# kekeblom/DeepCGP

Measured on AMD Instinct MI355X. Metric: ELBO steps/sec (batch=32) + achieved HBM GB/s on K_uf, MNIST M=256 1-layer, higher is better.
Workload: dtype f64; 1 GPU; cfg2_mnist_CH_M256; variant=conv layer + head, M=256, per_gpu_batch=32, global_batch=32, num_samples=10, layers=2, noise=device Philox RNG, dedup_layer0=False, parallelism=image-sharded x1, no collective

## Files before the change

### deepcgp_amd/csrc/common.h

```cpp
#pragma once
#include <hip/hip_runtime.h>
#include <cstdint>
#include <cstdio>
#include <map>
#include <string>
#include <vector>

#include "../../include/dcgp.h"
#include "dev_guard.h"
#include "fused_plan.h"

typedef double d4 __attribute__((ext_vector_type(4)));

static inline int round_up(int x, int m) { return (x + m - 1) / m * m; }
static inline long round_up_l(long x, long m) { return (x + m - 1) / m * m; }
long col_ld(long columns);

struct TimingAcc {
  int launches = 0;
  double ms = 0.0;
};
struct PendingEvent {
  std::string name;
  hipEvent_t start, stop;
};

struct DcgpOptions {
  long no_fused_layer = 0;
  long fused_large = 0;
  long fused_shape = -1;
  long fused_split = -1;
  long fused_persist = -1;
  long fused_pre = -1;
  long fused_parts = -1;
  long fused_rep_share = -1;
  long head_ride = -1;
  long fused_wgs = 0;
  long fused_stagger = -1;
  long kl_side = 0;
  long sweep_no_rows = 0;
  long kl_no_ride = 0;
  long no_fused_bwd = 0;
  long fused_bwd_min_cols = -1;
  long fused_bwd_frags = 0;
  long gemm_tile = 0;
  long grad_no_keep_k = 0;
  long grad_late_kl = 0;
  long head_unfused = 0;
  long no_side_stream = 0;
  long cu_partition = 0;
  long grad_nofork = 0;
  long head_no_overlap = 0;
  long no_factor_reuse = 0;
  long prep_on_chain = 0;
  long no_early_sweep = 0;
  long chain_no_iso = 0;
  long comm_inline = 0;
  long no_rhs_ride = 0;
  long kuf_upw = 0;
  long kuf_split = -1;
  long kuf_wpg = 0;
  long kuf_stream = 0;
  long kuf_no_rep = 0;
  long grad_dz_main = 0;
  long no_syrk = 0;
  long head_upw = 0;
  long share_kb = 0;
  long sweep_occ = -1;
  long head_tail = -1;
  long fused_abl = 0, rb_mixed = 0;
};
long* dcgp_option_slot(DcgpOptions* o, const char* name);
bool dcgp_poison(const char* name = nullptr);
size_t dcgp_guard_bytes();
struct dcgp_ctx;
hipError_t dev_alloc(dcgp_ctx* ctx, void** p, size_t bytes, const char* label);
void dev_free(dcgp_ctx* ctx, void* p);

struct dcgp_ctx {
  int device = 0;
  int n_cus = 256;
  hipStream_t stream = nullptr;
  hipStream_t stream2 = nullptr;
  hipStream_t stream2b = nullptr;
  hipStream_t stream_aux = nullptr;
  hipStream_t stream_comm = nullptr;
  hipEvent_t ev_comm[4] = {};
  int* comm_gate = nullptr;
  hipStream_t stream_m = nullptr, stream2_m = nullptr;
  hipStream_t last_main = nullptr;
  hipEvent_t ev_last = nullptr;
  bool ev_last_valid = false;
  hipEvent_t ev_fork = nullptr, ev_kl = nullptr;
  DcgpOptions opt;
  bool no_side = false;
  hipEvent_t ev_kl2 = nullptr, ev_kl3 = nullptr;
  hipEvent_t ev_g[6] = {};
  hipEvent_t ev_aux = nullptr, ev_aux2 = nullptr;
  std::string err;
  int last_head_rows = 0; long head_ride_launches = 0;
  unsigned fused_head_epoch = 0;
  unsigned fused_pre_epoch = 0;
  std::string ws_tag;
  std::map<std::string, std::pair<void*, size_t>> ws;
  dev_guard::Registry guards;
  bool timing = false;
  int timing_mode = 0;
  unsigned timing_sample = 0;
  std::map<std::string, TimingAcc> tim;
  std::vector<PendingEvent> pending;
  std::vector<hipEvent_t> event_pool;
  double* h_scratch = nullptr;
  int* h_info = nullptr;
  fused_plan::Plan last_fused_plan;
  long long* fused_trace = nullptr;
  std::string sweep_trace_family;
  long long* sweep_trace = nullptr; long sweep_trace_wgs = 0;
  void* comm = nullptr;
  int nranks = 1, rank = 0;
};

int ctx_fail(dcgp_ctx* ctx, int code, const char* fmt, ...);
void* ws_get(dcgp_ctx* ctx, const std::string& name, size_t bytes);
void timing_flush(dcgp_ctx* ctx);

#define HIP_TRY(ctx, call)                                                               \
  do {                                                                                   \
    hipError_t e_ = (call);                                                              \
    if (e_ != hipSuccess)                                                                \
      return ctx_fail((ctx), DCGP_ERR_HIP, "%s failed: %s (%s:%d)", #call, hipGetErrorString(e_), \
                      __FILE__, __LINE__);                                               \
  } while (0)

#define DCGP_TRY(call)        \
  do {                        \
    int s_ = (call);          \
    if (s_ != DCGP_OK) return s_; \
  } while (0)

#define LAUNCH_CHECK(ctx)                                                                \
  do {                                                                                   \
    hipError_t e_ = hipGetLastError();                                                   \
    if (e_ != hipSuccess)                                                                \
      return ctx_fail((ctx), DCGP_ERR_HIP, "kernel launch failed: %s (%s:%d)",           \
                      hipGetErrorString(e_), __FILE__, __LINE__);                        \
  } while (0)

struct ScopedTimer {
  dcgp_ctx* ctx;
  bool on;
  PendingEvent pe;
  ScopedTimer(dcgp_ctx* c, const char* name);
  ~ScopedTimer();
};


struct GemmArgs {
  const double* Wt = nullptr; long wBatch = 0; int ldw = 0;
  const double* B = nullptr;  long bBatch = 0; int ldb = 0;
  double* C = nullptr;        long cBatch = 0; int ldc = 0;
  double* colsq = nullptr;    long sBatch = 0; long sRowBlk = 0;
  const double* cscale = nullptr; long csCol = 0, csBatch = 0; double calpha = 1.0;
  int Mi = 0, Mk = 0, Kc = 0;
  int nW = 1, nB = 1;
  int tri = 0;
  int b_lower = 0;
  int rb_major = 0;
};
int gemm_tn(dcgp_ctx* ctx, const GemmArgs& a, int* n_row_blocks_out);
int gemm_row_block(int Mi, int Kc, int batch);

__device__ __forceinline__ double exp_sweep(double x) {
  const double kf = rint(x * 1.4426950408889634074);
  double r = fma(-kf, 6.93147180369123816490e-01, x);
  r = fma(-kf, 1.90821492927058770002e-10, r);
  double p = 1.6059043836821613e-10;
#define DCGP_EXP_STEP(c) asm("v_fma_f64 %0, %1, %2, %3" : "=v"(p) : "v"(p), "v"(r), "s"((double)(c)))
  DCGP_EXP_STEP(2.08767569878681e-09);
  DCGP_EXP_STEP(2.505210838544172e-08);
  DCGP_EXP_STEP(2.755731922398589e-07);
  DCGP_EXP_STEP(2.7557319223985893e-06);
  DCGP_EXP_STEP(2.48015873015873e-05);
  DCGP_EXP_STEP(1.984126984126984e-04);
// ... 192 lines not shown
```

### deepcgp_amd/csrc/conv_fused.hip

```cpp
#include <cstring>
#include <tuple>

#include "fused_plan.h"
#include "head_units_dev.h"
#include "layer.h"
#include "rng.h"

namespace {

typedef unsigned int u32x2 __attribute__((ext_vector_type(2)));
#define CF_SB __builtin_amdgcn_sched_barrier(0)
#define CF_DW 2
#define CF_P1 50
#define CF_P2 75
#define CF_P3 90
constexpr int CF_D_DEFAULT = 3;

__device__ __forceinline__ void set_prio(int p) {
  switch (p) {
    case 0: __builtin_amdgcn_s_setprio(0); break;
    case 1: __builtin_amdgcn_s_setprio(1); break;
    case 2: __builtin_amdgcn_s_setprio(2); break;
    default: __builtin_amdgcn_s_setprio(3); break;
  }
}
__device__ __forceinline__ int fdiv(int i, int d, float inv_d) {
  int q = (int)(((float)i + 0.5f) * inv_d);
  const int r = i - (int)__umul24((unsigned)q, (unsigned)d);
  return q + (r >= d ? 1 : 0) - (r < 0 ? 1 : 0);
}
__device__ __forceinline__ int frag_of(int w, int W, int c) { return (c >> 1) * 2 * W + ((c & 1) ? 2 * W - 1 - w : w); }

#define CF_TR(k) \
  if (tr_slot >= 0 && lane == 0) a.trace[(tr_slot * 16 + wave) * 16 + (k)] = (long long)__builtin_readcyclecounter();

template <int FN, int NS, int MAXF, int NT, int BTP, int ABL = 0, int HEAD = 0>
__global__ __launch_bounds__(NT) void conv_fused_kernel(ConvFusedArgs a_in) {
  constexpr int BT = BTP == 1 ? 1 : (BTP == 3 ? 2 : (BTP == 4 ? 3 : 0));
  typedef const __attribute__((address_space(4))) ConvFusedArgs KArgs;
  KArgs* ap = (KArgs*)__builtin_amdgcn_kernarg_segment_ptr();
  KArgs& a = *ap;
  constexpr int BN = FN * 16, W = NT / 64, TW = W / NS, FNS = FN / NS, KG = W / FN;
  static_assert(FN % NS == 0 && W % NS == 0 && W % FN == 0, "team split");
  constexpr int CF_D = ((ABL & 4) ? 2 : 0) + (NT >= 1024 ? CF_DW : CF_D_DEFAULT);
  extern __shared__ __attribute__((aligned(16))) double smem[];

  int cu_word = -1;
  if (a.persist && a.cu_slots) {
    int* word = reinterpret_cast<int*>(smem);
    if (threadIdx.x == 0) {
      unsigned xcc, hwid;
      asm volatile("s_getreg_b32 %0, hwreg(HW_REG_XCC_ID)" : "=s"(xcc));
      asm volatile("s_getreg_b32 %0, hwreg(HW_REG_HW_ID)" : "=s"(hwid));
      cu_word = (int)(((xcc & 7u) << 7) | ((hwid >> 8) & 0x7fu));
      word[0] = atomicAdd(a.cu_slots + cu_word, 1);
    }
    __syncthreads();
    const int arrival = word[0];
    __syncthreads();
    if ((arrival & 1) && a.stagger > 0) {
      const long long t0 = wall_clock64();
      while (wall_clock64() - t0 < a.stagger) __builtin_amdgcn_s_sleep(64);
    }
  }
  int strip_next = blockIdx.x;
  if (HEAD || a.pre_n > 0) {
    int* tk = reinterpret_cast<int*>(smem);
    if (threadIdx.x == 0) tk[0] = atomicAdd(a.dyn, 1);
    __syncthreads();
    strip_next = __builtin_amdgcn_readfirstlane(tk[0]);
    __syncthreads();
  }
  const int first_limit = HEAD ? a.n_items + a.head_n : (a.pre_n > 0 ? a.n_items : 0x7fffffff);
  for (int it = 0; strip_next < first_limit; ++it) {
  int tid = threadIdx.x;
  asm volatile("" : "+s"(ap), "+v"(tid));
  KArgs& a = *ap;
  if constexpr (HEAD) {
    if (strip_next >= a.n_items) {
      int* tk = reinterpret_cast<int*>(smem + a.lds_main + a.lds_img + BN);
      const int row = strip_next - a.n_items;
      if (tid == 0) {
        const int s_hi = (row * a.P + a.P - 1) / BN;
        int ok = 1;
        for (int st = (row * a.P) / BN; st <= s_hi && ok; ++st) {
          ok = 0;
          for (int spin = 0; spin < (1 << 24) && !ok; ++spin) {
            ok = __hip_atomic_load(a.head_flag + st, __ATOMIC_RELAXED, __HIP_MEMORY_SCOPE_AGENT) == a.head_epoch ? 1 : 0;
            if (!ok) __builtin_amdgcn_s_sleep(2);
          }
        }
        tk[1] = ok;
      }
      __syncthreads();
      if (tk[1]) {
        head_units_dev::head_units_body<0, 50, 0, NT, true>(ap->head, row);
      } else {
        for (int m = tid; m < a.head.kzx_rows; m += NT) a.head.kzx[(long)m * a.head.ldk + row] = __builtin_nan("");
      }
      if (tid == 0) tk[0] = atomicAdd(a.dyn, 1);
      __syncthreads();
      strip_next = __builtin_amdgcn_readfirstlane(tk[0]);
      if (strip_next >= first_limit) break;
      continue;
    }
  }
  const int Mp = a.Mp, nf = Mp >> 4, R = a.R;
  const int lane = tid & 63, lrow = lane >> 4, lcol = lane & 15;
  const int wave = __builtin_amdgcn_readfirstlane(tid >> 6);
  const int wm = wave % TW, sp = NS == 1 ? 0 : wave / TW;
  double* strip = smem;
  double* aux = smem + a.lds_main;
  double* xn = aux + a.lds_img;
  int* ticket = reinterpret_cast<int*>(xn + BN);
  int* koff = reinterpret_cast<int*>(xn + BN + 2);
  const int jmax = a.Kc - 1;
  int nfw = 0;
#pragma unroll
  for (int c = 0; c < MAXF; ++c) nfw += frag_of(wm, TW, c) < nf ? 1 : 0;
  nfw = __builtin_amdgcn_readfirstlane(nfw);
  int fr[MAXF];
#pragma unroll
  for (int c = 0; c < MAXF; ++c) fr[c] = c < nfw ? frag_of(wm, TW, c) : min(wm, nf - 1);
  int sidx = strip_next, sq = 0, SQ = 1;
  if (sidx >= a.split_first) {
    const int t = sidx - a.split_first;
    SQ = a.split_q;
    sidx = a.split_first + t / SQ;
    sq = t - (sidx - a.split_first) * SQ;
  }
  bool pre_fail = false;
  int mode = 0, pre_slot = 0;
  if (a.pre_D > 0) {
    if (strip_next < a.pre_D) { mode = 3; pre_slot = strip_next; }
    else if (strip_next >= a.pre_whole) { mode = 2; pre_slot = strip_next % a.pre_D; }
  } else if (a.pre_n > 0) {
    if (strip_next >= a.n_strips) {
      mode = 2;
      const int t = strip_next - a.n_strips;
      SQ = a.pre_sq;
      pre_slot = SQ > 1 ? t / SQ : t;
      sq = t - pre_slot * SQ;
      sidx = a.pre_first + pre_slot;
    }
    else if (strip_next >= a.pre_first && strip_next < a.pre_first + a.pre_n) { mode = 1; pre_slot = strip_next - a.pre_first; }
  }
  const int j0 = sidx * BN;
  int tr_slot = -1;
  if (a.trace) {
    const int every = a.persist ? max((int)gridDim.x / 8, 1) : 90;
    if (blockIdx.x % every == 0 && blockIdx.x / every < 8 && it < 4) tr_slot = (blockIdx.x / every) * 4 + it;
  }
  CF_TR(0)
  if (tr_slot >= 0 && lane == 0) a.trace[(tr_slot * 16 + wave) * 16 + 10] = (long long)wall_clock64();
  __builtin_amdgcn_s_setprio(3);

  unsigned voff[4];
#pragma unroll
  for (int q = 0; q < 4; ++q) voff[q] = (unsigned)(((4 * q + lrow) * Mp + lcol) * 8);
  auto ldw = [&](const __amdgpu_buffer_rsrc_t& rs, int soff, double (&dst)[4]) {
#pragma unroll
    for (int q = 0; q < 4; ++q) {
      const u32x2 v = __builtin_amdgcn_raw_buffer_load_b64(rs, (int)voff[q], soff, 0);
      __builtin_memcpy(&dst[q], &v, 8);
    }
  };
  constexpr int QS = 4 * BN;
  if (mode != 2) {
  const int n_first = j0 / a.P;
  const int n_last = min(j0 + BN - 1, jmax) / a.P;
  {
    const int total = (n_last - n_first + 1) * a.HWC;
    for (int i0 = 0; i0 < total; i0 += 4 * NT) {
      double t[4];
#pragma unroll
      for (int e = 0; e < 4; ++e) {
        const int i = i0 + e * NT + tid;
        const int n = fdiv(i, a.HWC, a.inv_HWC), o = i - n * a.HWC;
        const int nn = n_first + n, img = nn - fdiv(nn, a.n_mod, a.inv_nmod) * a.n_mod;
        t[e] = (i < total) ? a.X[(long)img * a.HWC + o] : 0.0;
      }
// ... 487 lines not shown
  }
  {
    const int y = wave % FN, g = wave / FN;
#pragma unroll
    for (int v = 0; v < 4; ++v) mup[(g * 16 + lrow + 4 * v) * BN + y * 16 + lcol] = macc[v];
  }
  __syncthreads();

  CF_TR(8)
  RngMap rmap;
  rmap.W = a.rmap.W; rmap.Nl = a.rmap.Nl; rmap.Ng = a.rmap.Ng; rmap.lo = a.rmap.lo;
  for (int idx = tid; idx < BN * R; idx += NT) {
    const int c = fdiv(idx, R, a.inv_R), r = idx - c * R;
    const int j = j0 + c;
    if (j > jmax || (SQ > 1 && r % SQ != sq)) continue;
    double s1 = 0.0, s2 = 0.0, m = 0.0;
    for (int w = 0; w < TW; ++w) {
      s1 += s1p[w * BN + c];
      s2 += s2p[(w * R + r) * BN + c];
    }
    for (int g = 0; g < KG; ++g) m += mup[(g * 16 + r) * BN + c];
    const double v = (a.knn - s1) + s2;
    if (pre_fail) m = __builtin_nan("");
    if (a.idm && r == 0) {
      const int n = j / a.P, p = j - n * a.P;
      const int oh = p / a.Wo, ow = p - oh * a.Wo, c0 = a.f / 2;
      m += a.X[(((long)(n % a.n_mod) * a.H + oh * a.s + c0) * a.W + ow * a.s + c0) * a.C];
    }
    const long e = (long)j * R + r;
    for (int s = 0; s < a.rep; ++s) {
      const long o = (long)s * a.rep_stride + e;
      if (a.out_mean) a.out_mean[o] = m;
      if (a.out_var) a.out_var[o] = v;
      if (a.out_sample) {
        const double zz = a.z ? a.z[o] : philox_normal(a.seed, a.stream_id, rng_index(rmap, o));
        const double smp = m + zz * sqrt(v + a.jitter);
        if constexpr (HEAD) __hip_atomic_store(a.out_sample + o, smp, __ATOMIC_RELAXED, __HIP_MEMORY_SCOPE_AGENT);
        else a.out_sample[o] = smp;
      }
    }
  }
  CF_TR(9)
  }
  if (tr_slot >= 0 && lane == 0) a.trace[(tr_slot * 16 + wave) * 16 + 11] = (long long)wall_clock64();
  if (!a.persist) break;
  if (tid == 0) ticket[0] = a.dyn ? ((HEAD || a.pre_n > 0) ? 0 : (int)gridDim.x) + atomicAdd(a.dyn, 1) : strip_next + (int)gridDim.x;
  if constexpr (HEAD) __builtin_amdgcn_s_waitcnt(0);
  __syncthreads();
  if constexpr (HEAD) {
    if (mode != 1 && tid == 0) __hip_atomic_store(a.head_flag + sidx, a.head_epoch, __ATOMIC_RELAXED, __HIP_MEMORY_SCOPE_AGENT);
  }
  strip_next = __builtin_amdgcn_readfirstlane(ticket[0]);
  if (strip_next >= (HEAD ? first_limit : a.n_items)) break;
  }
  if (threadIdx.x == 0) {
    if (cu_word >= 0) atomicSub(ap->cu_slots + cu_word, 1);
    if (ap->persist && ap->dyn && atomicAdd(ap->dyn + 1, 1) == (int)gridDim.x - 1) {
      ap->dyn[1] = 0;
      __threadfence();
      atomicExch(ap->dyn, 0);
    }
  }
}

using fused_plan::kShapes;
using fused_plan::Plan;
using fused_plan::Query;

template <int I, int BTP, int HEAD = 0>
int launch_instance(dcgp_ctx* ctx, const ConvFusedArgs& a, const Plan& p) {
  constexpr int FN = kShapes[I].FN, NS = kShapes[I].NS, MAXF = kShapes[I].MAXF, NT = kShapes[I].NT;
  static bool attr_done[64] = {};
  const int dv = ctx->device >= 0 && ctx->device < 64 ? ctx->device : 0;
  if (!attr_done[dv]) {
    hipFuncSetAttribute((const void*)conv_fused_kernel<FN, NS, MAXF, NT, BTP, 0, HEAD>, hipFuncAttributeMaxDynamicSharedMemorySize, 160 * 1024);
    attr_done[dv] = true;
  }
  hipLaunchKernelGGL((conv_fused_kernel<FN, NS, MAXF, NT, BTP, 0, HEAD>), dim3((unsigned)p.grid), dim3(NT), (size_t)p.lds, ctx->stream, a);
  LAUNCH_CHECK(ctx);
  return DCGP_OK;
}
template <int I>
int launch_fused(dcgp_ctx* ctx, const ConvFusedArgs& a, const Plan& p) {
  if (a.head_n > 0) {
    if constexpr (I == 0) {
      if (!p.patch_rows && a.bk.type == 0) return launch_instance<0, 0, 1>(ctx, a, p);
    }
    return ctx_fail(ctx, DCGP_ERR_ARG, "conv_fused: head rows on a launch that cannot carry them (shape %d)", I);
  }
  switch (p.patch_rows ? -1 : a.bk.type) {
    case 0: return launch_instance<I, 0>(ctx, a, p);
    case 1: return launch_instance<I, 1>(ctx, a, p);
    case 2: return launch_instance<I, 3>(ctx, a, p);
    case 3: return launch_instance<I, 4>(ctx, a, p);
    case -1:
      if constexpr (I == 0) return launch_instance<I, 2>(ctx, a, p);
      [[fallthrough]];
    default: return ctx_fail(ctx, DCGP_ERR_ARG, "conv_fused: unknown base kernel type %d", a.bk.type);
  }
}

Query fused_query(const dcgp_ctx* ctx, const ConvFusedArgs& a) {
  const DcgpOptions& o = ctx->opt;
  Query q;
  q.Mp = a.Mp; q.M = a.M; q.R = a.R; q.Rp = a.Rp; q.Kc = a.Kc; q.P = a.P; q.HWC = a.HWC; q.L = a.L; q.Lp = a.Lp; q.Lz = a.Lz; q.f = a.f; q.C = a.C;
  q.n_mod = a.n_mod; q.rep = a.rep; q.base = a.bk.type;
  q.has_G = a.G != nullptr; q.keeps_state = a.Kuf_out || a.A1_out; q.has_trace = ctx->fused_trace != nullptr; q.n_cus = ctx->n_cus;
  q.fused_shape = o.fused_shape; q.fused_large = o.fused_large; q.fused_split = o.fused_split; q.fused_persist = o.fused_persist; q.fused_pre = o.fused_pre;
  q.fused_parts = o.fused_parts; q.fused_rep_share = o.fused_rep_share; q.fused_wgs = o.fused_wgs; q.fused_stagger = o.fused_stagger;
  q.sweep_no_rows = o.sweep_no_rows;
  return q;
}

template <class T>
int ws_zeroed(dcgp_ctx* ctx, const char* name, size_t bytes, T** out, bool clear = false, bool* cleared = nullptr) {
  const auto it = ctx->ws.find(name);
  clear = clear || it == ctx->ws.end() || it->second.second < bytes;
  *out = static_cast<T*>(ws_get(ctx, name, bytes));
  if (!*out) return DCGP_ERR_ALLOC;
  if (clear) HIP_TRY(ctx, hipMemsetAsync(*out, 0, ctx->ws[name].second, ctx->stream));
  if (cleared) *cleared = clear;
  return DCGP_OK;
}

}

extern "C" int dcgp_debug_set_fused_trace(dcgp_ctx* ctx, long long* buf_dev) {
  if (!ctx) return DCGP_ERR_ARG;
  ctx->fused_trace = buf_dev;
  return DCGP_OK;
}

extern "C" int dcgp_debug_fused_plan(dcgp_ctx* ctx, int* out4) {
  if (!ctx || !out4) return DCGP_ERR_ARG;
  const Plan& p = ctx->last_fused_plan;
  out4[0] = p.persist; out4[1] = p.n_items; out4[2] = p.pre_n; out4[3] = p.pre_D;
  return DCGP_OK;
}

extern "C" int dcgp_debug_head_ride(dcgp_ctx* ctx, long long* out2) {
  if (!ctx || !out2) return DCGP_ERR_ARG;
  out2[0] = ctx->last_head_rows; out2[1] = ctx->head_ride_launches;
  return DCGP_OK;
}

extern "C" int dcgp_debug_plan_head_ride(const long long* query, int n_query, const long long* ride, int n_ride, long long row, long long* out, int n_out) {
  if (!query || !ride || !out || n_query != Query::kFields || n_ride != fused_plan::RideQuery::kFields || n_out != 8) return DCGP_ERR_ARG;
  Query q;
  std::apply([&](auto&... f) { ((f = (long)*query++), ...); }, Query::fields(q));
  fused_plan::RideQuery r;
  r.next_is_head = ride[0]; r.head_form = ride[1]; r.head_HWC = ride[2]; r.head_lds = ride[3]; r.head_nfm = ride[4]; r.in_flight = ride[5]; r.chain_beside = ride[6];
  r.head_ride = ride[7];
  const Plan p = fused_plan::plan_layer_launch(q);
  const fused_plan::Ride rd = fused_plan::plan_head_ride(q, p, r);
  long lo = 0, hi = -1, last = -1;
  if (rd.ok && row >= 0 && row < rd.n_rows) {
    fused_plan::ride_row_strips(row, q.P, kShapes[p.shape].FN * 16, &lo, &hi);
    for (long st = lo; st <= hi; ++st) last = std::max(last, fused_plan::ride_sample_item(p, st));
  }
  const long long flat[8] = {rd.ok, rd.why, rd.n_rows, rd.first_item, rd.ok ? rd.first_item + row : -1, lo, hi, last};
  memcpy(out, flat, sizeof flat);
  return DCGP_OK;
}

extern "C" int dcgp_debug_plan_layer_launch(const long long* query, int n_query, long long* plan, int n_plan) {
  if (!query || !plan || n_query != Query::kFields || n_plan != Plan::kFields) return DCGP_ERR_ARG;
  Query q;
  auto fields = Query::fields(q);
  static_assert(std::tuple_size<decltype(fields)>::value == Query::kFields, "the flat query covers every field");
  std::apply([&](auto&... f) { ((f = (long)*query++), ...); }, fields);
  const Plan p = fused_plan::plan_layer_launch(q);
  long long units[3];
  const double u[3] = {p.units_plain, p.units_ahead, p.units_shared};
  memcpy(units, u, sizeof units);
  const long long flat[Plan::kFields] = {p.ok, p.shape, p.lds, p.lds_main, p.lds_img, p.grid, p.persist, p.n_strips, p.n_items, p.deal, p.split_first, p.split_q,
                                         p.pre_n, p.pre_first, p.pre_sq, p.pre_D, p.pre_whole, p.pre_stride, p.stagger, p.cu_slots, p.patch_rows,
                                         units[0], units[1], units[2]};
  memcpy(plan, flat, sizeof flat);
  return DCGP_OK;
}

bool conv_fused_ok(const dcgp_ctx* ctx, const ConvFusedArgs& a) {
  return !ctx->opt.no_fused_layer && fused_plan::plan_layer_launch(fused_query(ctx, a)).ok;
}

int conv_fused_rides_head(const dcgp_ctx* ctx, const ConvFusedArgs& a, bool keeps_state, bool head_form, long head_HWC, long head_lds, long head_nfm, bool in_flight,
                           bool chain_beside) {
  if (ctx->opt.no_fused_layer) return 0;
  Query q = fused_query(ctx, a);
  q.keeps_state = keeps_state;
  fused_plan::RideQuery r;
  r.next_is_head = 1; r.head_form = head_form; r.head_HWC = head_HWC; r.head_lds = head_lds; r.head_nfm = head_nfm; r.in_flight = in_flight;
  r.chain_beside = chain_beside; r.head_ride = ctx->opt.head_ride;
  return fused_plan::plan_head_ride(q, fused_plan::plan_layer_launch(q), r).n_rows;
}

int conv_fused(dcgp_ctx* ctx, const ConvFusedArgs& a_in) {
  if (a_in.Kc <= 0) return DCGP_OK;
  const Plan p = fused_plan::plan_layer_launch(fused_query(ctx, a_in));
  if (!p.ok) return ctx_fail(ctx, DCGP_ERR_ARG, "conv_fused: layer shape not supported (M = %d, R = %d)", a_in.M, a_in.R);
  ConvFusedArgs a = a_in;
  if (p.deal == fused_plan::kCounter) DCGP_TRY(ws_zeroed(ctx, "fused_dyn", 2 * sizeof(int), &a.dyn));
  if (p.pre_n > 0) {
    a.pre_buf = static_cast<double*>(ws_get(ctx, "fused_pre_buf", (size_t)p.pre_n * p.pre_stride * sizeof(double)));
    if (!a.pre_buf) return DCGP_ERR_ALLOC;
    bool cleared = false;
    DCGP_TRY(ws_zeroed(ctx, "fused_pre_flag", (size_t)p.pre_n * sizeof(unsigned), &a.pre_flag, ctx->fused_pre_epoch == 0xffffffffu, &cleared));
    if (cleared) ctx->fused_pre_epoch = 0;
    a.pre_epoch = ++ctx->fused_pre_epoch;
  }
  if (p.cu_slots) DCGP_TRY(ws_zeroed(ctx, "fused_cu_slots", 1024 * sizeof(int), &a.cu_slots));
  ctx->last_head_rows = 0;
  if (a.head_n > 0) {
    fused_plan::RideQuery rq;
    rq.next_is_head = 1; rq.head_form = 1; rq.head_HWC = a.head.HWC; rq.head_lds = (long)head_units_lds(a.head); rq.head_nfm = a.head.nfm;
    rq.head_ride = ctx->opt.head_ride;
    const fused_plan::Ride ride = fused_plan::plan_head_ride(fused_query(ctx, a_in), p, rq);
    if (!ride.ok || ride.n_rows != a.head_n || a.head.X != a.out_sample || a.head.N != a_in.Kc / a_in.P || a.head.n_mod < a.head.N || a.head.n0 != 0 || !a.head.kzx ||
        a.head.kuf || a.head.kfull || a.head.trace)
      return ctx_fail(ctx, DCGP_ERR_ARG, "conv_fused: the launch cannot carry the head's rows (reason %d)", ride.why);
    a.head.kd = nullptr; a.head.want_kd = 0;
    a.head.nseg = 1; a.head.seg[0] = HuSeg{}; a.head.n_wgs = a.head_n; a.head.upw = 1;
    bool cleared = false;
    DCGP_TRY(ws_zeroed(ctx, "fused_head_flag", (size_t)p.n_strips * sizeof(unsigned), &a.head_flag, ctx->fused_head_epoch == 0xffffffffu, &cleared));
    if (cleared) ctx->fused_head_epoch = 0;
    a.head_epoch = ++ctx->fused_head_epoch;
    ctx->last_head_rows = a.head_n;
    ++ctx->head_ride_launches;
  }
  a.lds_main = p.lds_main; a.lds_img = p.lds_img;
  a.split_first = p.split_first; a.split_q = p.split_q;
  a.persist = p.persist; a.n_strips = p.n_strips; a.n_items = p.n_items; a.stagger = p.stagger;
  a.pre_n = p.pre_n; a.pre_first = p.pre_first; a.pre_sq = p.pre_sq; a.pre_stride = p.pre_stride; a.pre_D = p.pre_D; a.pre_whole = p.pre_whole;
  a.trace = ctx->fused_trace;
  a.no_rows = ctx->opt.sweep_no_rows ? 1 : 0;
  a.inv_HWC = 1.0f / (float)a.HWC; a.inv_nmod = 1.0f / (float)a.n_mod; a.inv_P = 1.0f / (float)a.P; a.inv_Wo = 1.0f / (float)a.Wo; a.inv_R = 1.0f / (float)a.R;
  ctx->last_fused_plan = p;
  ScopedTimer t(ctx, "conv_fused");
#ifdef DCGP_EXPERIMENTS
  const int abl = (int)ctx->opt.fused_abl;
  if (abl && p.shape == 0 && a.bk.type == 0) {
    const unsigned grid = (unsigned)((a.Kc + 63) / 64);
#define CF_ABL(X)                                                                                                                       \
  case X:                                                                                                                               \
    hipFuncSetAttribute((const void*)conv_fused_kernel<4, 2, 2, 1024, 0, X>, hipFuncAttributeMaxDynamicSharedMemorySize, 160 * 1024); \
    hipLaunchKernelGGL((conv_fused_kernel<4, 2, 2, 1024, 0, X>), dim3(grid), dim3(1024), (size_t)p.lds, ctx->stream, a);               \
    break;
    switch (abl) { CF_ABL(1) CF_ABL(2) CF_ABL(3) CF_ABL(4) default: return ctx_fail(ctx, DCGP_ERR_ARG, "conv_fused: unknown DCGP_FUSED_ABL value %d", abl); }
#undef CF_ABL
    LAUNCH_CHECK(ctx);
    return DCGP_OK;
  }
#endif
  static_assert(fused_plan::kNumShapes == 8, "one case per row of the shape table");
  switch (p.shape) {
    case 0: return launch_fused<0>(ctx, a, p);
    case 1: return launch_fused<1>(ctx, a, p);
    case 2: return launch_fused<2>(ctx, a, p);
    case 3: return launch_fused<3>(ctx, a, p);
    case 4: return launch_fused<4>(ctx, a, p);
    case 5: return launch_fused<5>(ctx, a, p);
    case 6: return launch_fused<6>(ctx, a, p);
    default: return launch_fused<7>(ctx, a, p);
  }
}
```

### deepcgp_amd/csrc/ctx.hip

```cpp
#include <cctype>
#include <cstdarg>
#include <cstdlib>
#include <cstring>

#include "common.h"

int ctx_fail(dcgp_ctx* ctx, int code, const char* fmt, ...) {
  char buf[1024];
  va_list ap;
  va_start(ap, fmt);
  vsnprintf(buf, sizeof(buf), fmt, ap);
  va_end(ap);
  if (ctx) ctx->err = buf;
  return code;
}

namespace {
struct OptSlot { const char* name; long DcgpOptions::*field; };
const OptSlot kOptSlots[] = {
    {"no_fused_layer", &DcgpOptions::no_fused_layer}, {"fused_large", &DcgpOptions::fused_large}, {"fused_shape", &DcgpOptions::fused_shape}, {"fused_split", &DcgpOptions::fused_split},
    {"kl_side", &DcgpOptions::kl_side}, {"kl_no_ride", &DcgpOptions::kl_no_ride}, {"sweep_no_rows", &DcgpOptions::sweep_no_rows}, {"no_fused_bwd", &DcgpOptions::no_fused_bwd}, {"fused_bwd_min_cols", &DcgpOptions::fused_bwd_min_cols},
    {"fused_bwd_frags", &DcgpOptions::fused_bwd_frags}, {"grad_late_kl", &DcgpOptions::grad_late_kl}, {"gemm_tile", &DcgpOptions::gemm_tile}, {"grad_no_keep_k", &DcgpOptions::grad_no_keep_k},
    {"head_unfused", &DcgpOptions::head_unfused}, {"no_side_stream", &DcgpOptions::no_side_stream}, {"cu_partition", &DcgpOptions::cu_partition},
    {"grad_nofork", &DcgpOptions::grad_nofork}, {"head_no_overlap", &DcgpOptions::head_no_overlap},
    {"no_early_sweep", &DcgpOptions::no_early_sweep}, {"prep_on_chain", &DcgpOptions::prep_on_chain}, {"no_factor_reuse", &DcgpOptions::no_factor_reuse}, {"kuf_upw", &DcgpOptions::kuf_upw},
    {"no_rhs_ride", &DcgpOptions::no_rhs_ride}, {"comm_inline", &DcgpOptions::comm_inline}, {"chain_no_iso", &DcgpOptions::chain_no_iso}, {"kuf_no_rep", &DcgpOptions::kuf_no_rep}, {"kuf_stream", &DcgpOptions::kuf_stream},
    {"kuf_wpg", &DcgpOptions::kuf_wpg}, {"kuf_split", &DcgpOptions::kuf_split}, {"head_tail", &DcgpOptions::head_tail},
    {"sweep_occ", &DcgpOptions::sweep_occ}, {"share_kb", &DcgpOptions::share_kb}, {"head_upw", &DcgpOptions::head_upw}, {"no_syrk", &DcgpOptions::no_syrk}, {"grad_dz_main", &DcgpOptions::grad_dz_main},
    {"fused_persist", &DcgpOptions::fused_persist}, {"fused_stagger", &DcgpOptions::fused_stagger}, {"fused_pre", &DcgpOptions::fused_pre}, {"fused_parts", &DcgpOptions::fused_parts},
    {"fused_rep_share", &DcgpOptions::fused_rep_share}, {"fused_wgs", &DcgpOptions::fused_wgs}, {"head_ride", &DcgpOptions::head_ride},
    {"fused_abl", &DcgpOptions::fused_abl}, {"rb_mixed", &DcgpOptions::rb_mixed},
};
}
long* dcgp_option_slot(DcgpOptions* o, const char* name) {
  for (const OptSlot& s : kOptSlots)
    if (strcmp(s.name, name) == 0) return &(o->*s.field);
  return nullptr;
}

static void options_from_env(DcgpOptions* o) {
  for (const OptSlot& s : kOptSlots) {
    std::string e = "DCGP_";
    for (const char* c = s.name; *c; ++c) e += (char)toupper((unsigned char)*c);
    const char* v = getenv(e.c_str());
    if (!v) continue;
    char* end = nullptr;
    const long x = strtol(v, &end, 10);
    o->*s.field = (end != v) ? x : 1;
  }
}

bool dcgp_poison(const char* name) {
  static const bool poison = getenv("DCGP_POISON_WS") != nullptr;
  static const char* only = getenv("DCGP_POISON_ONLY");
  return poison && (!name || !only || strstr(name, only) != nullptr);
}

size_t dcgp_guard_bytes() {
  static const size_t guard = dev_guard::parse_bytes(getenv("DCGP_GUARD_WS"));
  return guard;
}

static hipError_t dev_alloc_cap(dcgp_ctx* ctx, void** p, size_t bytes, size_t cap, const char* label) {
  const size_t guard = dcgp_guard_bytes();
  const size_t total = guard ? bytes + guard : cap;
  const hipError_t e = hipMalloc(p, total);
  if (e != hipSuccess) { *p = nullptr; return e; }
  const bool poison = dcgp_poison(label);
  if (poison) hipMemset(*p, 0xFF, guard ? bytes : cap);
  if (guard) {
    hipMemset((char*)*p + bytes, 0xFF, guard);
    if (ctx) ctx->guards.add(*p, bytes, label);
  }
  if (poison || guard) hipDeviceSynchronize();
  return hipSuccess;
}
hipError_t dev_alloc(dcgp_ctx* ctx, void** p, size_t bytes, const char* label) { return dev_alloc_cap(ctx, p, bytes, bytes, label); }

static long guard_scan_device(const void* p, const dev_guard::Entry& e) {
  std::vector<unsigned char> h(dcgp_guard_bytes());
  if (hipMemcpy(h.data(), (const char*)p + e.bytes, h.size(), hipMemcpyDeviceToHost) != hipSuccess) return 0;
  return dev_guard::scan(h.data(), h.size());
}

void dev_free(dcgp_ctx* ctx, void* p) {
  if (!p) return;
  dev_guard::Entry e;
  if (dcgp_guard_bytes() && ctx && ctx->guards.remove(p, &e)) {
    hipDeviceSynchronize();
    const long off = guard_scan_device(p, e);
    if (off >= 0) ctx->guards.remember(e, off);
  }
  hipFree(p);
}

void* ws_get(dcgp_ctx* ctx, const std::string& name, size_t bytes) {
  if (bytes == 0) bytes = 16;
  auto it = ctx->ws.find(name);
  if (it != ctx->ws.end() && it->second.second >= bytes) return it->second.first;
  if (it != ctx->ws.end()) {
    hipDeviceSynchronize();
    dev_free(ctx, it->second.first);
    ctx->ws.erase(it);
  }
  void* p = nullptr;
  size_t cap = dcgp_guard_bytes() ? bytes : (bytes + 255) / 256 * 256;
  if (dev_alloc_cap(ctx, &p, bytes, cap, name.c_str()) != hipSuccess) {
    ctx_fail(ctx, DCGP_ERR_ALLOC, "workspace '%s': allocation of %zu bytes failed", name.c_str(), cap);
    return nullptr;
  }
  ctx->ws[name] = {p, cap};
  return p;
}
// ... 326 lines not shown
```

### deepcgp_amd/csrc/fused_plan.h

```cpp
#pragma once
#include <algorithm>
#include <functional>
#include <map>
#include <mutex>
#include <queue>
#include <tuple>
#include <vector>

namespace fused_plan {

struct FusedShape { int FN, NS, MAXF, NT, max_nf; };
constexpr FusedShape kShapes[] = {{4, 2, 2, 1024, 16}, {4, 1, 2, 512, 16}, {2, 1, 2, 512, 16}, {1, 1, 2, 512, 16},
                                  {2, 1, 2, 768, 24},  {2, 1, 2, 1024, 32}, {1, 1, 4, 1024, 64},
                                  {2, 2, 2, 1024, 16}};
constexpr int kNumShapes = sizeof(kShapes) / sizeof(kShapes[0]);
constexpr long kLdsBytes = 160 * 1024;

struct Query {
  long Mp = 0, M = 0, R = 0, Rp = 0, Kc = 0, P = 0, HWC = 0, L = 0, Lp = 0, Lz = 0, f = 0, C = 0, n_mod = 0, rep = 1;
  long base = 0;
  long has_G = 0;
  long keeps_state = 0;
  long has_trace = 0;
  long n_cus = 0;
  long fused_shape = -1, fused_large = 0, fused_split = -1, fused_persist = -1, fused_pre = -1, fused_parts = -1, fused_rep_share = -1, fused_wgs = 0,
       fused_stagger = -1, sweep_no_rows = 0;
  static constexpr int kFields = 29;
  template <class Q>
  static auto fields(Q& q) {
    return std::tie(q.Mp, q.M, q.R, q.Rp, q.Kc, q.P, q.HWC, q.L, q.Lp, q.Lz, q.f, q.C, q.n_mod, q.rep, q.base, q.has_G, q.keeps_state, q.has_trace, q.n_cus,
                    q.fused_shape, q.fused_large, q.fused_split, q.fused_persist, q.fused_pre, q.fused_parts, q.fused_rep_share, q.fused_wgs, q.fused_stagger,
                    q.sweep_no_rows);
  }
  bool operator<(const Query& o) const { return fields(*this) < fields(o); }
};

enum Deal { kPerStrip = 0, kCounter = 1, kFixedStride = 2 };

struct Plan {
  int ok = 0;
  int shape = 0;
  long lds = 0;
  int lds_main = 0, lds_img = 0;
  long grid = 0;
  int persist = 0;
  int n_strips = 0, n_items = 0;
  int deal = kPerStrip;
  int split_first = 1 << 30, split_q = 1;
  int pre_n = 0, pre_first = 0, pre_sq = 1, pre_D = 0, pre_whole = 0;
  long pre_stride = 0;
  int stagger = 0;
  int cu_slots = 0;
  int patch_rows = 0;
  double units_plain = 0.0, units_ahead = 0.0, units_shared = 0.0;
  static constexpr int kFields = 24;
};

constexpr double kCostPrologue = 1.75, kCostEpilogue = 0.3, kCostHandOver = 0.2;
constexpr double kDealMargin = 0.98;
constexpr double kShareMargin = 0.9;
constexpr double kFront = 0.11;
constexpr double kEps = 1e-9;

enum Item { kWhole, kLeaving, kPrologueOnly, kConsumer };
class DealSim {
 public:
  DealSim(long slots, long R, long handovers) : R_((double)R), ready_((size_t)std::max<long>(handovers, 0), 0.0) {
    for (long i = 0; i < slots; ++i) free_at_.push(0.0);
  }
  void give(Item kind, long slot = 0, double outputs = 0.0) {
    const double F = kCostPrologue + R_ + kCostEpilogue;
    if (kind == kWhole) run(F, 0.0);
    else if (kind == kLeaving) ready_[(size_t)slot] = run(F + kCostHandOver, 0.0) - (R_ + kCostEpilogue);
    else if (kind == kPrologueOnly) ready_[(size_t)slot] = run(kCostPrologue + kCostHandOver, 0.0);
    else run(kCostHandOver + outputs + kCostEpilogue, ready_[(size_t)slot]);
  }
  double makespan() const { return end_; }
  std::vector<double> free_times() const {
    std::vector<double> out;
    for (auto q = free_at_; !q.empty(); q.pop()) out.push_back(q.top());
    return out;
  }

 private:
  double run(double cost, double not_before) {
    const double t = std::max(free_at_.top(), not_before) + cost;
    free_at_.pop();
    free_at_.push(t);
    end_ = std::max(end_, t);
    return t;
  }
  double R_, end_ = 0.0;
  std::vector<double> ready_;
  std::priority_queue<double, std::vector<double>, std::greater<double>> free_at_;
};

inline double ahead_units(long strips, long slots, long first, long n_pre, long R, long SQ = 1, int NS = 1) {
  DealSim d(slots, R, n_pre);
  for (long i = 0; i < first; ++i) d.give(kWhole);
  for (long i = 0; i < n_pre; ++i) d.give(kPrologueOnly, i);
  for (long i = 0; i < strips - first - n_pre; ++i) d.give(kWhole);
  for (long i = 0; i < n_pre; ++i)
    for (long q = 0; q < SQ; ++q) {
      const long nr = q < R ? (R - 1 - q) / SQ + 1 : 0;
      d.give(kConsumer, i, SQ == 1 ? (double)R : (double)(NS * ((nr + NS - 1) / NS)));
    }
  return d.makespan();
}
inline double shared_units(long strips, long slots, long D, long whole, long R) {
  DealSim d(slots, R, D);
  for (long i = 0; i < strips; ++i) {
    if (i < D) d.give(kLeaving, i);
    else if (i < whole) d.give(kWhole);
    else d.give(kConsumer, i % D, (double)R);
  }
  return d.makespan();
}

inline double last_round(const Query& q, const FusedShape& sh, long strips, long slots, int* q_out) {
  *q_out = 1;
  const long want = q.fused_split, R = q.R;
  const long rem = strips % slots;
  if (rem == 0) return 0.0;
  if (want == 0 || want == 1 || sh.NT != 1024 || !q.has_G || R < 2) return 1.0;
  const long whole = (R + sh.NS - 1) / sh.NS;
  const long qmax = std::min(slots / rem, R);
  double best = kShareMargin;
  for (long s = 2; s <= qmax; ++s) {
    const long part = ((R + s - 1) / s + sh.NS - 1) / sh.NS;
    const double cost = kFront + (1.0 - kFront) * (double)part / (double)whole;
    if ((want > 1 && s <= want) || (want < 0 && cost < best - kEps)) { best = cost; *q_out = (int)s; }
  }
  return *q_out > 1 ? best : 1.0;
}

inline Plan plan_uncached(const Query& q) {
  Plan p;
  const long nf = q.Mp / 16;
  if (q.Rp != 16 || q.R > 16 || q.R < 1 || q.Mp > 1024 || q.Mp < 16 || q.Mp % 16 || q.P <= 0) return p;
  if (q.Kc >= (1 << 23) || q.HWC >= (1 << 23)) return p;
  const long force = q.fused_shape;
  if (nf > 16 && force < 0 && !q.fused_large) return p;
  const long all_cus = q.n_cus > 0 ? q.n_cus : 256;

  double best = 0.0;
  int shape_q = 1;
  for (int i = 0; i < kNumShapes; ++i) {
    const FusedShape& sh = kShapes[i];
    if (force >= 0 && i != force) continue;
    if (nf > sh.max_nf) continue;
    if (sh.max_nf > 16 && nf <= 16 && force < 0) continue;
    if (i == 1 && force < 0) continue;
    const long BN = sh.FN * 16, W = sh.NT / 64, TW = W / sh.NS, KG = W / sh.FN;
    const long nimg = (BN - 1) / q.P + 2;
    const long main_d = std::max(q.Mp * BN, (TW * q.R + KG * 16) * BN);
    const long img_d = std::max((nimg * q.HWC + 1) & ~1L, TW * BN);
    const long bytes = (main_d + img_d + BN + 2) * 8 + std::max(q.Lz, q.Lp) * 4;
    if (bytes > kLdsBytes) continue;
    const long strips = q.Kc > 0 ? (q.Kc + BN - 1) / BN : 1;
// ... 48 lines not shown
    return p;
  }
  p.persist = (int)(per_cu * slots);
  p.grid = p.persist;
  p.n_strips = p.n_items = (int)strips;
  p.deal = want != 2 ? kCounter : kFixedStride;
  if (per_cu > 1) {
    p.stagger = (int)((q.fused_stagger >= 0 ? q.fused_stagger : 40) * 100);
    p.cu_slots = 1;
  }
  if (per_cu != 1 || p.deal != kCounter || !q.has_G) return p;

  const long stride = q.Mp * BN + TW * BN;
  if (parts > 1) {
    p.pre_n = (int)strips; p.pre_sq = (int)parts; p.pre_stride = stride;
    p.n_items = (int)(strips + strips * parts);
    return p;
  }
  const long S = p.persist;
  p.units_plain = (double)((strips + S - 1) / S) * whole_strip;
  long n_pre = 0;
  const long rem = strips % S, rounds = strips / S, pre = q.fused_pre;
  if (pre != 0 && rem != 0 && rounds >= 1 && rounds <= 16 && R >= 2) {
    const long per = pre > 0 ? pre : (long)(whole_strip / (kCostPrologue + kCostHandOver));
    const long most = std::min((S - rem) * per, strips - rem), step = std::max<long>(S / 8, 1);
    double best_t = p.units_plain * (pre > 0 ? 2.0 : kDealMargin);
    for (long n = step; n <= most; n += step) {
      const double t = ahead_units(strips, S, rem, n, R);
      if (t < best_t - kEps) { best_t = t; n_pre = n; p.units_ahead = t; }
    }
  }
  long D = 0;
  if (q.fused_rep_share != 0 && pre < 0 && q.n_mod > 0 && q.rep == 1 && q.Kc % q.P == 0 && !q.keeps_state) {
    const long rows = q.Kc / q.P, period = q.n_mod * q.P;
    if (rows % q.n_mod == 0 && rows / q.n_mod >= 2 && period % BN == 0) D = period / BN;
    if (D >= strips || D > 4 * S) D = 0;
  }
  if (D > 0) {
    p.pre_whole = (int)std::max(D, std::min(S, strips));
    p.units_shared = shared_units(strips, S, D, p.pre_whole, R);
    const double today = n_pre > 0 ? std::min(p.units_plain, p.units_ahead) : p.units_plain;
    if (!(p.units_shared < today * kDealMargin - kEps)) D = p.pre_whole = 0;
  }
  if (D > 0) {
    p.pre_n = p.pre_D = (int)D;
    p.pre_stride = stride;
  } else if (n_pre > 0) {
    p.pre_n = (int)n_pre;
    p.pre_first = (int)rem;
    p.n_items = (int)(strips + n_pre);
    p.pre_stride = stride;
  }
  return p;
}

inline Plan plan_layer_launch(const Query& q) {
  static std::mutex mu;
  static std::map<Query, Plan> memo;
  std::lock_guard<std::mutex> lock(mu);
  const auto it = memo.find(q);
  if (it != memo.end()) return it->second;
  if (memo.size() > 256) memo.clear();
  return memo[q] = plan_uncached(q);
}

struct RideQuery {
  long next_is_head = 0;
  long head_form = 0;
  long head_HWC = 0;
  long head_lds = 0;
  long head_nfm = 0;
  long in_flight = 0;
  long chain_beside = 0;
  long head_ride = -1;
  static constexpr int kFields = 8;
};
enum RideWhy { kRides = 0, kRideOff, kRideNotHead, kRideForm, kRideLaunch, kRideState, kRideTrace, kRideInFlight, kRideGeometry, kRideNoRoom };
struct Ride {
  int ok = 0, why = kRideOff;
  int n_rows = 0;
  int first_item = 0;
};
constexpr double kCostHeadRow = 3.0;
inline long ride_room(const Query& q, const Plan& p) {
  const long S = p.persist, strips = p.n_strips, R = q.R;
  DealSim d(S, R, p.pre_n);
  if (p.pre_D > 0) {
    for (long i = 0; i < strips; ++i) {
      if (i < p.pre_D) d.give(kLeaving, i);
      else if (i < p.pre_whole) d.give(kWhole);
      else d.give(kConsumer, i % p.pre_D, (double)R);
    }
  } else if (p.pre_n > 0) {
    for (long i = 0; i < p.pre_first; ++i) d.give(kWhole);
    for (long i = 0; i < p.pre_n; ++i) d.give(kPrologueOnly, i);
    for (long i = 0; i < strips - p.pre_first - p.pre_n; ++i) d.give(kWhole);
    for (long i = 0; i < p.pre_n; ++i) d.give(kConsumer, i, (double)R);
  } else {
    for (long i = 0; i < strips; ++i) d.give(kWhole);
  }
  long room = 0;
  for (double t : d.free_times()) room += (long)((d.makespan() - t + kEps) / kCostHeadRow);
  return room;
}
inline Ride plan_head_ride(const Query& q, const Plan& p, const RideQuery& r) {
  Ride out;
  auto no = [&](int why) { out.ok = 0; out.why = why; return out; };
  if (r.head_ride == 0) return no(kRideOff);
  if (!r.next_is_head) return no(kRideNotHead);
  if (!r.head_form) return no(kRideForm);
  if (!p.ok || p.shape != 0 || p.persist <= 0 || p.deal != kCounter || p.grid != p.persist || p.cu_slots || p.patch_rows || q.base != 0 || q.rep != 1 ||
      p.pre_sq != 1 || p.split_q != 1)
    return no(kRideLaunch);
  if (q.keeps_state) return no(kRideState);
  if (q.has_trace) return no(kRideTrace);
  if (r.in_flight || r.chain_beside) return no(kRideInFlight);
  if (q.P <= 0 || q.Kc <= 0 || q.Kc % q.P || q.P * q.R != r.head_HWC || r.head_nfm < 1 || r.head_nfm > kShapes[0].NT / 64 || r.head_lds > (long)p.lds_main * 8)
    return no(kRideGeometry);
  const long rows = q.Kc / q.P;
  const long n = r.head_ride > 0 ? std::min(r.head_ride, rows) : std::min(ride_room(q, p), rows);
  if (n <= 0) return no(kRideNoRoom);
  out.ok = 1; out.why = kRides;
  out.n_rows = (int)n;
  out.first_item = p.n_items;
  return out;
}
inline void ride_row_strips(long row, long P, long BN, long* lo, long* hi) { *lo = row * P / BN; *hi = (row * P + P - 1) / BN; }
inline long ride_sample_item(const Plan& p, long strip) {
  if (p.pre_n > 0 && p.pre_D == 0 && strip >= p.pre_first && strip < p.pre_first + p.pre_n) return p.n_strips + (strip - p.pre_first) * p.pre_sq;
  return strip;
}

}
```

### deepcgp_amd/csrc/head_units_dev.h

```cpp
#pragma once
#include "common.h"
#include <cmath>
#include <type_traits>

namespace head_units_dev {

typedef unsigned int u32x2 __attribute__((ext_vector_type(2)));
constexpr int kOob = (int)0x80000000u;

__device__ __forceinline__ int fdiv_small(int i, float inv_d) { return (int)(((float)i + 0.5f) * inv_d); }

#ifndef HU_SB1
#define HU_SB1 __builtin_amdgcn_sched_barrier(0)
#endif
#ifndef HU_WAVES
#define HU_WAVES 4
#endif
#ifndef HU_EXPN
#define HU_EXPN 4
#endif
#define HU_LDX(i) (COH ? __hip_atomic_load(Xn + (i), __ATOMIC_RELAXED, __HIP_MEMORY_SCOPE_AGENT) : Xn[i])
template <int NK4, int TL, int WMODE, int NT, bool COH = false>
__device__ __forceinline__ void head_units_body(const __attribute__((address_space(4))) HeadUnitsArgs& a, const int block) {
  extern __shared__ __attribute__((aligned(16))) double smem[];
  constexpr bool WRITE = WMODE == 1 || WMODE == 2;
  constexpr bool KEEP = WMODE == 3;
  constexpr int WPG = NT / 64;
  constexpr bool RES = NK4 > 0;
  constexpr int NKR = RES ? NK4 : 1;
  constexpr int RW = RES ? 0 : TL;
  constexpr int RL = (NK4 == 7 && TL == 1) ? 5 : ((NK4 == 5 && TL == 0) ? 4 : ((NK4 == 13 && TL == 0) ? 12 : 0));
  constexpr bool PERM = RL > 0;
  const int HWC = a.HWC, L = a.L, nk4 = RES ? NK4 : a.Lq >> 2, nfp = a.nfp, P = a.P, np16 = nfp * 16;
  const int HWCe = (HWC + 1) & ~1;
  double* img = smem;
  double* xb = img + HWCe;
  double* wl = xb + np16;
  double* rs = wl + np16;
  int* pbl = reinterpret_cast<int*>(rs + ((a.H * (a.W - a.f + 1) + 1) & ~1));
  int* koff = pbl + np16;
  double* etab = reinterpret_cast<double*>(koff + ((a.Lq + 1) & ~1));
  const char* imgb = reinterpret_cast<const char*>(img);
  const int tid = threadIdx.x, lane = tid & 63, lrow = lane >> 4, lcol = lane & 15;
  const int wave = __builtin_amdgcn_readfirstlane(tid >> 6);
  int sg = 0;
#pragma unroll
  for (int q = 1; q < 6; ++q)
    if (q < a.nseg && block >= a.seg[q].wg0) sg = q;
  const int seg_kind = a.seg[sg].kind, seg_T = a.seg[sg].T, seg_C = a.seg[sg].C;
  const int wloc = block - a.seg[sg].wg0, wpi = a.seg[sg].wpi;
  const int nloc = wloc / wpi, bw = wloc - nloc * wpi;
  const int n = a.seg[sg].img0 + nloc;
  const double* __restrict__ Xn = a.X + (long)((a.n0 + n) % a.n_mod) * HWC;
  auto ldi = [&](int byte_off) { return *reinterpret_cast<const double*>(imgb + byte_off); };
  long long* const tr = (a.trace && block < a.trace_wgs) ? a.trace + ((long)block * WPG + wave) * 8 : nullptr;
  auto stamp = [&](int k) { if (tr && lane == 0) tr[k] = (long long)clock64(); };
  if (tr && lane == 0) {
    unsigned xcc, hwid;
    asm volatile("s_getreg_b32 %0, hwreg(HW_REG_XCC_ID)" : "=s"(xcc));
    asm volatile("s_getreg_b32 %0, hwreg(HW_REG_HW_ID)" : "=s"(hwid));
    tr[0] = (long long)wall_clock64();
    tr[7] = (long long)(((xcc & 0xf) << 16) | (hwid & 0xffff)) << 32;
  }
  stamp(1);

  {
    constexpr int IB = NT <= 128 ? 16 : 8;
    double t[IB];
#pragma unroll
    for (int e = 0; e < IB; ++e) {
      const int i = e * NT + tid;
      t[e] = (i < HWC) ? HU_LDX(i) : 0.0;
    }
    if (RES)
      for (int i = tid; i < 256; i += NT) etab[i] = a.exp_tab[i];
    for (int l = tid; l < a.Lq; l += NT) {
      const int ll = l < L ? l : 0;
      const int tq = fdiv_small(ll, a.inv_C), c = ll - tq * a.C;
      const int kh = fdiv_small(tq, a.inv_f), kw = tq - kh * a.f;
      koff[l] = ((kh * a.W + kw) * a.C + c) * 8;
    }
    for (int p = tid; p < np16; p += NT) {
      const int q = p < P ? p : 0;
      const int oh = fdiv_small(q, a.inv_Wo), ow = q - oh * a.Wo;
      pbl[p] = (oh * a.s * a.W + ow * a.s) * a.C * 8;
      wl[p] = (!WRITE && p < P) ? a.w[p] : 0.0;
    }
#pragma unroll
    for (int e = 0; e < IB; ++e) {
      const int i = e * NT + tid;
      if (i < HWC) img[i] = t[e] * a.csq;
    }
    for (int i0 = IB * NT; i0 < HWC; i0 += IB * NT) {
#pragma unroll
      for (int e = 0; e < IB; ++e) {
        const int i = i0 + e * NT + tid;
        t[e] = (i < HWC) ? HU_LDX(i) : 0.0;
      }
#pragma unroll
      for (int e = 0; e < IB; ++e) {
        const int i = i0 + e * NT + tid;
        if (i < HWC) img[i] = t[e] * a.csq;
      }
    }
  }
  __syncthreads();
  stamp(2);
  {
    const int Wr = a.W - a.f + 1, fC = a.f * a.C;
    for (int i = tid; i < a.H * Wr; i += NT) {
      const int r = fdiv_small(i, a.inv_Wr), x = i - r * Wr;
      const double* src = img + (r * a.W + x) * a.C;
      double acc = 0.0;
      int j = 0;
      for (; j + 4 <= fC; j += 4) {
        const double v0 = src[j], v1 = src[j + 1], v2 = src[j + 2], v3 = src[j + 3];
        acc = fma(v0, v0, acc); acc = fma(v1, v1, acc); acc = fma(v2, v2, acc); acc = fma(v3, v3, acc);
      }
      for (; j < fC; ++j) acc = fma(src[j], src[j], acc);
      rs[i] = acc;
    }
    __syncthreads();
    for (int p = tid; p < np16; p += NT) {
      const int q = p < P ? p : 0;
      const int oh = fdiv_small(q, a.inv_Wo), ow = q - oh * a.Wo;
      const double* src = rs + oh * a.s * Wr + ow * a.s;
      double acc = 0.0;
      int kh = 0;
      for (; kh + 4 <= a.f; kh += 4) {
        const double v0 = src[kh * Wr], v1 = src[(kh + 1) * Wr], v2 = src[(kh + 2) * Wr], v3 = src[(kh + 3) * Wr];
        acc += (v0 + v1) + (v2 + v3);
      }
      for (; kh < a.f; ++kh) acc += src[kh * Wr];
      xb[p] = -0.5 * acc;
    }
  }
  __syncthreads();

  stamp(3);
  const int seg_upw = a.seg[sg].upw;
  int u = WPG * seg_upw * bw + ((wave + n) & (WPG - 1));
  const int n_units = seg_kind == 1 ? seg_C : (WRITE ? a.nfm * a.st_split : a.nfm);
  if (u >= n_units) {
    if (tr && lane == 0) tr[6] = (long long)wall_clock64();
    return;
  }

  const int sL = RES ? NK4 - (TL == 3 ? 2 : 1) : L >> 2;
  double tB_real[2], tB_nrm[2], tB_one[2];
#pragma unroll
  for (int ts = 0; ts < 2; ++ts) {
    const int k = 4 * (sL + ts) + lrow;
    tB_real[ts] = k < L ? 1.0 : 0.0;
    tB_one[ts] = k == L ? 1.0 : 0.0;
    tB_nrm[ts] = k == L + 1 ? 1.0 : 0.0;
  }
  int kob[NKR];
  if (RES) {
#pragma unroll
    for (int s = 0; s < NKR; ++s) kob[s] = (PERM && s < RL) ? koff[RL * lrow] + 8 * s : koff[4 * s + lrow];
  }
  int kdel[2] = {0, 0};
  if (PERM) {
#pragma unroll
    for (int q = 0; q < 2; ++q) kdel[q] = RL + q < NKR ? kob[RL + q < NKR ? RL + q : 0] - kob[0] : 0;
  }
  static_assert(!PERM || NKR - RL <= 2, "at most two sub-steps behind the runs");
  auto pbx = [&](int frag) { const int p0 = pbl[16 * frag + lcol]; return PERM ? p0 + kob[0] : p0; };
  auto ld0 = [&](int pbv) { return PERM ? ldi(pbv) : ldi(pbv + (RES ? kob[0] : koff[lrow])); };
  auto ldB = [&](int pbv, int s) {
    if (PERM) return s < RL ? ldi(pbv + 8 * s) : ldi(pbv + kdel[s - RL < 1 ? 0 : 1]);
    return ldi(pbv + kob[RES ? s : 0]);
  };
  auto fixB = [&](double v, int s, double nrm) {
    const int ts = s - sL;
    const double t0 = ts ? tB_real[1] : tB_real[0], t1 = ts ? tB_nrm[1] : tB_nrm[0], t2 = ts ? tB_one[1] : tB_one[0];
    return fma(v, t0, fma(nrm, t1, t2));
  };
  auto fixA = [&](double v, int s, double nrm) {
    const int ts = s - sL;
    const double t0 = ts ? tB_real[1] : tB_real[0], t1 = ts ? tB_one[1] : tB_one[0], t2 = ts ? tB_nrm[1] : tB_nrm[0];
    return fma(v, t0, fma(nrm, t1, t2));
  };

  __amdgpu_buffer_rsrc_t st_rs = __builtin_amdgcn_make_buffer_rsrc(a.kuf, 0, 0, 0x00020000);
  int st_voff[4] = {kOob, kOob, kOob, kOob};
  bool st_zero = false;
  const int st_nrep = (WRITE && a.n_base < a.N) ? (a.N - 1 - n) / a.n_mod + 1 : 1;
  const bool st_hold = WMODE == 2 && st_nrep > 1 && a.st_hold;
  int ur = 0;

  int kd_pa = 0;
  auto group = [&](auto kd_tag, auto ny_tag, auto&& getA, auto&& getA_raw, int j0, int next_j0, int nyn, double* rdiag, double (&rsum)[4], int (&pb)[4], double (&bv)[4]) {
    constexpr int NY = decltype(ny_tag)::value;
    constexpr bool KD = decltype(kd_tag)::value;
    d4 acc[NY];
#pragma unroll
    for (int y = 0; y < NY; ++y) acc[y] = d4{0.0, 0.0, 0.0, 0.0};
    auto xbv = [&](int y) { return xb[16 * (j0 + y) + lcol]; };
    if (RES) {
#pragma unroll
      for (int s = 0; s < NKR; ++s) {
        double bn[NY];
        if (s + 1 < NKR) {
#pragma unroll
          for (int y = 0; y < NY; ++y) bn[y] = ldB(pb[y], s + 1);
        }
        HU_SB1;
        const double av = getA(s);
        if (s >= sL) {
#pragma unroll
          for (int y = 0; y < NY; ++y) bv[y] = fixB(bv[y], s, xbv(y));
        }
#pragma unroll
        for (int y = 0; y < NY; ++y) acc[y] = __builtin_amdgcn_mfma_f64_16x16x4f64(av, bv[y], acc[y], 0, 0, 0);
        if (s + 1 < NKR) {
#pragma unroll
          for (int y = 0; y < NY; ++y) bv[y] = bn[y];
        }
        __builtin_amdgcn_sched_barrier(0);
      }
    } else if constexpr (RW > 0) {
      static_assert(RW % 4 == 2, "patch rows of 4 n + 2 elements: two rows and the sub-step that straddles them are a period of 2 n + 1 sub-steps");
      constexpr int NA = RW / 4, DA = 5;
// ... 354 lines not shown
```

### deepcgp_amd/csrc/layer.h

```cpp
#pragma once
#include "common.h"
#include "rng.h"

struct ViewGeom {
  int H = 0, W = 0, C = 0, f = 0, s = 0, Ho = 0, Wo = 0, P = 0, L = 0;
  void set(int H_, int W_, int C_, int f_, int s_) {
    H = H_; W = W_; C = C_; f = f_; s = s_;
    Ho = (H - f) / s + 1; Wo = (W - f) / s + 1; P = Ho * Wo; L = f * f * C;
  }
};

struct GpMats {
  int M = 0, Mp = 0, R = 0, Rp = 0;
  double* K = nullptr;
  double* Linv = nullptr;
  double* LinvT = nullptr;
  double* Kp = nullptr;
  double* Lpinv = nullptr;
  double* LpinvT = nullptr;
  double* Lq = nullptr;
  double* qmu = nullptr;
  double* G = nullptr;
  double* alpha = nullptr;
  double* klp = nullptr;
// ... 7 lines not shown
};

struct PrepLayerArgs {
  const double *Z = nullptr, *Z0 = nullptr, *q_sqrt = nullptr, *q_mu = nullptr;
  double *K = nullptr, *Kp = nullptr, *ZT = nullptr, *zn = nullptr, *Lq = nullptr, *qmu = nullptr;
  int M = 0, Mp = 0, L = 0, Lp = 0, R = 0, Rp = 0;
  BaseKernel bk; double jitter = 0.0;
  const double* in_scale = nullptr;
  double* ZS = nullptr; int Lz = 0;
};
struct PrepArgs {
  int nl = 0;
  PrepLayerArgs l[8];
};
constexpr unsigned kPrepSweepTasks = (1u << 2) | (1u << 5);
int prepare_all(dcgp_ctx* ctx, const PrepArgs& a, unsigned task_mask = ~0u);

struct CondScratch {
  double *A1 = nullptr, *s1p = nullptr, *s2p = nullptr, *mu = nullptr;
  int nrb1 = 0, nrb3 = 0;
  long ldb = 0;
};
int cond_prep(dcgp_ctx* ctx, GpMats& g, int white, bool have_qsqrt);
int cond_core(dcgp_ctx* ctx, const GpMats& g, const double* B, long ldb, int Kc, int white, bool have_qsqrt,
              const char* ws_prefix, CondScratch* out, hipEvent_t prep_done = nullptr, bool head = false);

struct KlTail;
struct KlOffer { const KlTail* tail = nullptr; double* scal = nullptr; bool carried = false; };
bool head_cond_fused_ok(const GpMats& g);
int head_cond_fused(dcgp_ctx* ctx, const GpMats& g, const double* B, long ldb, int Kc, bool have_qsqrt, const double* kd,
                    double* out_mean, double* out_var, int kd_n = 1, double kd_scale = 1.0, double* A1_out = nullptr, long lda1 = 0, KlOffer* kl = nullptr);

int prep_solve_all(dcgp_ctx* ctx, GpMats* const* gs, const int* white, const bool* have_qsqrt, int nl, bool* done, const bool* skip = nullptr);

struct FinalizeArgs {
  const double* s1p = nullptr; int nrb1 = 0;
  const double* s2p = nullptr; int nrb3 = 0;
  const double* mu = nullptr;
  long ldk = 0;
  int Kc = 0, R = 0;
  long col0 = 0;
  double knn_scalar = 0.0; const double* knn_vec = nullptr;
  int rep = 1; long rep_stride = 0;
  const double* z = nullptr;
  uint64_t seed = 0; uint32_t stream_id = 0;
  RngMap rmap;
  double jitter = 0.0;
  double *out_sample = nullptr, *out_mean = nullptr, *out_var = nullptr;
  const double* X = nullptr; int idm = 0; int n_mod = 0; int H = 0, W = 0, C = 0, f = 0, s = 0, Wo = 0, P = 0;
};
int finalize_layer(dcgp_ctx* ctx, const FinalizeArgs& a);

struct ConvFusedArgs {
  const double* X = nullptr; int n_mod = 0;
  int H = 0, W = 0, C = 0, f = 0, s = 0, Wo = 0, P = 0, L = 0, Lp = 0, HWC = 0;
  const double* ZT = nullptr; const double* zn = nullptr; int M = 0, Mp = 0;
  const double* ZS = nullptr; int Lz = 0; double csq = 1.0;
  BaseKernel bk;
  const double* LinvT = nullptr;
  const double* G = nullptr;
  const double* alpha = nullptr; int R = 0, Rp = 0;
  int Kc = 0;
  double knn = 0.0;
  int rep = 1; long rep_stride = 0;
  const double* z = nullptr; uint64_t seed = 0; uint32_t stream_id = 0; double jitter = 0.0;
  RngMap rmap;
  double *out_sample = nullptr, *out_mean = nullptr, *out_var = nullptr;
  int idm = 0;
  double *Kuf_out = nullptr, *A1_out = nullptr; long ldk = 0;
  int lds_main = 0, lds_img = 0;
  float inv_HWC = 0, inv_nmod = 0, inv_P = 0, inv_Wo = 0, inv_R = 0;
  int split_first = 1 << 30, split_q = 1;
  long long* trace = nullptr;
  int persist = 0, n_strips = 0;
  int stagger = 0;
  int* dyn = nullptr;
  int* cu_slots = nullptr;
  int no_rows = 0;
  int pre_n = 0, pre_first = 0, pre_sq = 1; long pre_stride = 0;
  double* pre_buf = nullptr; unsigned* pre_flag = nullptr; unsigned pre_epoch = 0;
  int n_items = 0;
  int pre_D = 0, pre_whole = 0;
  int head_n = 0;
  unsigned* head_flag = nullptr; unsigned head_epoch = 0;
  HeadUnitsArgs head;
};
struct ConvBwdArgs {
  const double* A1 = nullptr; long ld = 0; int Kc = 0;
  const double* S = nullptr;
  const double* alpha = nullptr; int Rp = 0;
  const double* Linv = nullptr;
  const double *gv = nullptr, *gm = nullptr, *gvs = nullptr;
  int M = 0, Mp = 0, R = 0;
  double* dKuf = nullptr;
};
bool conv_bwd_fused_ok(const dcgp_ctx* ctx, const ConvBwdArgs& a);
int conv_bwd_fused(dcgp_ctx* ctx, const ConvBwdArgs& a);
bool conv_fused_ok(const dcgp_ctx* ctx, const ConvFusedArgs& a);
int conv_fused(dcgp_ctx* ctx, const ConvFusedArgs& a);
int conv_fused_rides_head(const dcgp_ctx* ctx, const ConvFusedArgs& a, bool keeps_state, bool head_form, long head_HWC, long head_lds, long head_nfm, bool in_flight,
                           bool chain_beside);

int kl_layer(dcgp_ctx* ctx, const GpMats& g, const double* Lp, const double* LpinvT, int white, const char* ws_prefix,
             double* kl4);

struct FactorStatus {
  const int* info[16];
  int ninfo[16];
  int ngroups = 0;
};
struct ElboFinish {
  int nl = 0;
  int M[8], R[8], white[8];
  double scale = 1.0;
  FactorStatus st;
  double* host_out = nullptr;
  double host_seq = 0.0;
};
struct TailArgs;
struct KlTailLayer {
  const double* Lfac = nullptr; long ldf = 0;
  const double* Lq = nullptr;
  const double* sums = nullptr;
  int ns = 0, nsa = 0;
  int M = 0, Mp = 0, R = 0;
};
struct KlTail { int nl = 0; KlTailLayer l[8]; };
int elbo_tail_prepare(dcgp_ctx* ctx, TailArgs* t);
int elbo_tail(dcgp_ctx* ctx, const double* mu, const double* var, const int32_t* y, int n_rows, int n_labels, int K, double eps,
              double* ve_rows, double inv_s, double* scal, const ElboFinish& fin, const KlTail* kl = nullptr);
int varexp_rows(dcgp_ctx* ctx, const double* mu, const double* var, const int32_t* y, int n_rows, int n_labels, int K,
                double eps, double* out_rows, int predict);
const double* gauss_hermite_table(dcgp_ctx* ctx);

constexpr int kEvalMaxSlots = 8192;
int eval_tail(dcgp_ctx* ctx, const double* mu, const double* var, const int32_t* y, int n, int S, int K, double eps, long lo,
              double* logdens, double* p_mean, int* ok);
int eval_sum(dcgp_ctx* ctx, const double* logdens, const int* ok, long n, const FactorStatus& st, double* res);

int gauss_elbo_tail(dcgp_ctx* ctx, const double* mu, const double* var, const double* y, int n_rows, int n_labels, int K, const double* s2,
                    double* ve_rows, double inv_s, double* scal, const ElboFinish& fin, const KlTail* kl = nullptr);
int gauss_grad(dcgp_ctx* ctx, const double* mu, const double* var, const double* y, int rows, int K, int n_labels, const double* s2,
               double weight, double* gm, double* gv, double* gs2);
int gauss_predict(dcgp_ctx* ctx, const double* mu, const double* var, long n, const double* s2, double* out_mean, double* out_var);
int gauss_eval_tail(dcgp_ctx* ctx, const double* mu, const double* var, const double* y, int n, int S, int K, const double* s2, long lo,
                    double* logdens, double* ld_nd, double* y_mean, double* sqerr);
int gauss_eval_sum(dcgp_ctx* ctx, const double* logdens, const double* sqerr, long n, const FactorStatus& st, double* res);

int bern_elbo_tail(dcgp_ctx* ctx, const double* mu, const double* var, const double* y, int n_rows, int n_labels, int K, double* ve_rows,
                   double inv_s, double* scal, const ElboFinish& fin, const KlTail* kl = nullptr);
int bern_grad(dcgp_ctx* ctx, const double* mu, const double* var, const double* y, int rows, int K, int n_labels, double weight, double* gm,
              double* gv);
int bern_predict(dcgp_ctx* ctx, const double* mu, const double* var, long n, double* out_mean, double* out_var);
int bern_eval_tail(dcgp_ctx* ctx, const double* mu, const double* var, const double* y, int n, int S, int K, long lo, double* logdens,
                   double* ld_nd, double* p_mean, double* correct);

struct QuadLik {
  int kind = 0;
  const double* scale = nullptr;
  double scale_val = 1.0, nu = 3.0, c_nu = 0.0, binsize = 1.0;
};
double student_t_const(double nu);
int quad_elbo_tail(dcgp_ctx* ctx, const QuadLik& q, const double* mu, const double* var, const double* y, int n_rows, int n_labels, int K,
                   double* ve_rows, double inv_s, double* scal, const ElboFinish& fin, const KlTail* kl = nullptr);
int quad_grad(dcgp_ctx* ctx, const QuadLik& q, const double* mu, const double* var, const double* y, int rows, int K, int n_labels, double weight,
              double* gm, double* gv, double* gpar);
int quad_predict(dcgp_ctx* ctx, const QuadLik& q, const double* mu, const double* var, long n, double* out_mean, double* out_var);
int quad_elementwise(dcgp_ctx* ctx, const QuadLik& q, int what, const double* mu, const double* var, const double* y, long n, double* out_a,
                     double* out_b);
int quad_eval_tail(dcgp_ctx* ctx, const QuadLik& q, const double* mu, const double* var, const double* y, int n, int S, int K, long lo,
                   double* logdens, double* ld_nd, double* y_mean, double* sqerr);

int softmax_elbo_tail(dcgp_ctx* ctx, const double* mu, const double* var, const int32_t* y, int n_rows, int n_labels, int K, const double* nodes, int Q,
                      double* ve_rows, double inv_s, double* scal, const ElboFinish& fin, const KlTail* kl = nullptr);
int softmax_grad(dcgp_ctx* ctx, const double* mu, const double* var, const int32_t* y, int rows, int n_labels, int K, const double* nodes, int Q,
                 double weight, double* gm, double* gv);
int softmax_predict(dcgp_ctx* ctx, const double* mu, const double* var, int rows, int K, const double* nodes, int Q, double* out_mean, double* out_var);
int softmax_eval_tail(dcgp_ctx* ctx, const double* mu, const double* var, const int32_t* y, int n, int S, int K, const double* nodes, int Q, long lo,
                      double* logdens, double* p_mean, int* ok);
struct UncOut;
int softmax_unc_tail(dcgp_ctx* ctx, const double* mu, const double* var, const int32_t* y, int n, int S, int K, const double* nodes, int Q, long lo,
                     const UncOut& o);
int softmax_density_grad(dcgp_ctx* ctx, const double* mu, const double* var, const int32_t* y, int n_img, int S, int K, const double* nodes, int Q,
                         double* J, double* gm, double* gv);
// ... 68 lines not shown
```

### deepcgp_amd/csrc/layer_impl.h

```cpp
#pragma once
#include <cstdlib>
#include <cstring>
#include <memory>
#include <string>

#include "layer.h"

int additive_kdiag_async(dcgp_ctx* ctx, int N, int P, double variance, const double* w, double* out_N);
int reparam_async(dcgp_ctx* ctx, const double* mean, const double* var, const double* z, size_t n, double jitter,
                  double* out);
int allreduce_sum_f64_async(dcgp_ctx* ctx, double* buf_dev, int n);
struct LayerState;
int conv_mean_add(dcgp_ctx* ctx, const LayerState& L, const double* X, int n_mod, long col0, long Kc, int rep, long rep_stride, double* out_mean,
                  double* out_sample);
int conv_mean_backward_dx(dcgp_ctx* ctx, const LayerState& L, const double* gm, int rows, double* dXin);
int conv_mean_backward_filter(dcgp_ctx* ctx, const LayerState& L, const double* Xcol, const double* gm, long Kc, double* gW);
constexpr int kMixMaxMaps = 64;
int mix_forward(dcgp_ctx* ctx, const double* W, int G, int R, const double* u, const double* gm, const double* gv, long col0, long Kc, int rep,
                long lat_stride, long out_stride, double* out_sample, double* out_mean, double* out_var);
int mix_backward_latent(dcgp_ctx* ctx, const double* W, int G, int R, const double* gF, long Kc, double* gu);
void mix_w_plan(long Kc, int* nwg, long* cpw);
int mix_backward_w(dcgp_ctx* ctx, int G, int R, const double* u, const double* gF, long Kc, double* part, double* gW);

struct LayerState {
// ... 210 lines not shown
    for (void* p : {(void*)dK, (void*)dLinv, (void*)dLinvT, (void*)d_info, (void*)d_rhs, (void*)d_yw}) dev_free(owner, p);
    dK = dLinv = dLinvT = nullptr; d_info = nullptr; d_rhs = nullptr; d_yw = nullptr; uploaded = false;
  }
  int upload(dcgp_ctx* ctx) {
    if (uploaded) return DCGP_OK;
    const size_t n = K.size();
    owner = ctx;
    if (dev_alloc(ctx, (void**)&dK, n * sizeof(double*), "fg_dK") != hipSuccess || dev_alloc(ctx, (void**)&dLinv, n * sizeof(double*), "fg_dLinv") != hipSuccess ||
        dev_alloc(ctx, (void**)&dLinvT, n * sizeof(double*), "fg_dLinvT") != hipSuccess || dev_alloc(ctx, (void**)&d_info, n * sizeof(int), "fg_info") != hipSuccess)
      return ctx_fail(ctx, DCGP_ERR_ALLOC, "factor group: allocation failed");
    HIP_TRY(ctx, hipMemcpy(dK, K.data(), n * sizeof(double*), hipMemcpyHostToDevice));
    HIP_TRY(ctx, hipMemcpy(dLinv, Linv.data(), n * sizeof(double*), hipMemcpyHostToDevice));
    HIP_TRY(ctx, hipMemcpy(dLinvT, LinvT.data(), n * sizeof(double*), hipMemcpyHostToDevice));
    if (ride) {
      size_t total = 0;
      for (auto& r : rhs) total += (r.Lq || r.qmu) ? (size_t)r.R * Mp * Mp + (size_t)Mp * r.Rp : 0;
      if (dev_alloc(ctx, (void**)&d_yw, (total ? total : 2) * sizeof(double), "fg_yw") != hipSuccess || dev_alloc(ctx, (void**)&d_rhs, n * sizeof(ChainRhs), "fg_rhs") != hipSuccess)
        return ctx_fail(ctx, DCGP_ERR_ALLOC, "factor group: allocation failed");
      size_t off = 0;
      for (auto& r : rhs) {
        r.Yw = d_yw + off;
        off += (r.Lq || r.qmu) ? (size_t)r.R * Mp * Mp + (size_t)Mp * r.Rp : 0;
      }
      HIP_TRY(ctx, hipMemcpy(d_rhs, rhs.data(), n * sizeof(ChainRhs), hipMemcpyHostToDevice));
    }
    uploaded = true;
    return DCGP_OK;
  }
  bool deferred = false;
  bool rode = false;
  int run(dcgp_ctx* ctx, bool defer_finish = false, ChainMode mode = ChainMode()) {
    DCGP_TRY(upload(ctx));
    rode = ride && chain_can_ride(ctx, Mp, mode);
    DCGP_TRY(factor_inverse_batched(ctx, dK, dLinv, dLinvT, (int)K.size(), Mp, Mp, d_info, defer_finish, rode ? d_rhs : nullptr, max_R, mode));
    deferred = defer_finish;
    return DCGP_OK;
  }
  int finish(dcgp_ctx* ctx) {
    if (!deferred) return DCGP_OK;
    deferred = false;
    return factor_finish_batched(ctx, dK, (int)K.size(), Mp, Mp);
  }
};

static inline ConvFusedArgs conv_fused_shape(const LayerState& L, long rows) {
  ConvFusedArgs fa;
  fa.H = L.v.H; fa.W = L.v.W; fa.C = L.v.C; fa.f = L.v.f; fa.s = L.v.s; fa.Wo = L.v.Wo; fa.P = L.v.P; fa.L = L.v.L; fa.Lp = L.Lp;
  fa.HWC = L.v.H * L.v.W * L.v.C;
  fa.ZT = L.ZT; fa.zn = L.zn; fa.M = L.M; fa.Mp = L.Mp; fa.bk = L.base();
  fa.ZS = L.ZS; fa.Lz = L.Lz; fa.csq = sqrt(1.4426950408889634074) / L.ls;
  fa.LinvT = L.g.LinvT; fa.G = L.has_qsqrt ? L.g.G : nullptr; fa.alpha = L.g.alpha; fa.R = L.R; fa.Rp = L.g.Rp;
  fa.Kc = (int)std::min<long>(rows * L.v.P, 0x7fffffffL); fa.knn = L.variance; fa.idm = L.identity_mean;
  if (L.in_scale) fa.P = 0;
  return fa;
}
static inline bool first_layer_one_launch(const dcgp_ctx* ctx, const LayerState& L, long rows) {
  return L.is_head ? !(L.Mp >= 96 && !ctx->opt.head_no_overlap) : conv_fused_ok(ctx, conv_fused_shape(L, rows));
}

static inline HeadUnitsArgs head_sweep_shape(const dcgp_ctx* ctx, const LayerState& L, const double* X, int rows, int n_mod, double* B, long ldb) {
  HeadUnitsArgs h;
  h.X = X; h.n_mod = n_mod; h.N = rows;
  h.H = L.v.H; h.W = L.v.W; h.C = L.v.C; h.f = L.v.f; h.s = L.v.s; h.Wo = L.v.Wo; h.P = L.v.P; h.L = L.v.L; h.Lq = L.Lz;
  h.ZS = L.ZS; h.M = L.M; h.Mp = L.Mp;
  h.csq = sqrt(1.4426950408889634074) / L.ls; h.log2var = log2(L.variance);
  h.w = L.w; h.kzx = B; h.ldk = ldb; h.kzx_scale = 1.0 / (double)L.v.P;
  h.want_kd = 1;
  h.tail_mode = (int)ctx->opt.head_tail;
  h.occ_force = (int)ctx->opt.sweep_occ;
  h.share_kb = (int)ctx->opt.share_kb;
  h.upw_force = (int)ctx->opt.head_upw;
  return h;
}
static inline bool head_takes_unit_sweep(const LayerState& L) { return L.is_head && L.kernel_type == 0 && L.base().type == 0 && !L.in_scale; }
static inline bool head_sweep_rides_form(const dcgp_ctx* ctx, const LayerState& L, const HeadUnitsArgs& h) {
  return head_takes_unit_sweep(L) && !h.kuf && !h.kfull && h.f * h.C == 50 && (h.f & 1) && h.L == h.f * h.f * h.C && !ctx->opt.sweep_no_rows &&
         h.Lq == round_up(h.L + 2, 4) && h.Mp % 16 == 0 && head_units_ok(h);
}

static inline int conv_forward(dcgp_ctx* ctx, LayerState& L, const double* X, int rows, int n_mod, int rep, long rep_stride,
                 const double* z, uint64_t seed, uint32_t stream_id, double jitter, double* out_sample, double* out_mean,
                 double* out_var, const std::string& pfx, hipEvent_t factor_done = nullptr,
                               hipEvent_t prep_done = nullptr, int phase = 3, bool keep_state = true, const RngMap* rmap = nullptr,
                               int planned_one_launch = -1, const HeadUnitsArgs* ride_head = nullptr, int ride_rows = 0) {
  const int Mp = L.Mp, P = L.v.P;
  const long Kc = (long)rows * P;
  if (Kc > 0x7fffff00L) return ctx_fail(ctx, DCGP_ERR_ARG, "conv layer: %ld patch columns exceed the 32-bit tile index", Kc);
  const long ldb = col_ld(Kc);
  const long out_stride = rep_stride / L.R * L.Rout;
  double *const mix_sample = out_sample, *const mix_mean = out_mean, *const mix_var = out_var;
  if (L.mix_W) {
    if (!L.lat_sample || L.lat_cap < (size_t)(rep > 1 ? (long)rep * rep_stride : Kc * L.R))
      return ctx_fail(ctx, DCGP_ERR_ARG, "conv layer: a mixed layer without its latent buffers");
    out_sample = L.lat_sample; out_mean = L.lat_mean; out_var = L.lat_var;
  }
  {
    ConvFusedArgs fa = conv_fused_shape(L, rows);
    fa.X = X; fa.n_mod = n_mod;
    fa.rep = rep; fa.rep_stride = rep_stride; fa.z = z; fa.seed = seed; fa.stream_id = stream_id; fa.jitter = jitter;
    fa.out_sample = out_sample; fa.out_mean = out_mean; fa.out_var = out_var;
    if (rmap) fa.rmap = *rmap;
    const bool one_launch = conv_fused_ok(ctx, fa);
    if (planned_one_launch >= 0 && one_launch != (planned_one_launch != 0))
      return ctx_fail(ctx, DCGP_ERR_ARG, "conv layer: the step was planned for the %s route, the layer takes the other (M = %d, %ld patch columns)",
                      planned_one_launch ? "one-launch" : "sweep + GEMM", L.M, Kc);
    if (one_launch) {
      if (!(phase & 2)) return DCGP_OK;
      if (keep_state) {
        fa.Kuf_out = (double*)ws_get(ctx, pfx + "Kuf", (size_t)Mp * ldb * sizeof(double));
        fa.A1_out = (double*)ws_get(ctx, pfx + "A1", (size_t)Mp * ldb * sizeof(double));
        if (!fa.Kuf_out || !fa.A1_out) return DCGP_ERR_ALLOC;
        fa.ldk = ldb;
      }
      if (prep_done) HIP_TRY(ctx, hipStreamWaitEvent(ctx->stream, prep_done, 0));
      else if (factor_done) HIP_TRY(ctx, hipStreamWaitEvent(ctx->stream, factor_done, 0));
      if (ride_head) { fa.head = *ride_head; fa.head_n = ride_rows; }
      if (!L.mean_W && !L.mix_W) return conv_fused(ctx, fa);
      if (ride_head && ride_rows > 0 && L.mix_W) return ctx_fail(ctx, DCGP_ERR_ARG, "conv layer: a mixed layer cannot carry the head's rows");
      if (ride_head && ride_rows > 0) return ctx_fail(ctx, DCGP_ERR_ARG, "conv layer: a layer with a mean filter cannot carry the head's rows");
      DCGP_TRY(conv_fused(ctx, fa));
      if (L.mix_W)
        DCGP_TRY(mix_forward(ctx, L.mix_W, L.R, L.Rout, out_sample, out_mean, out_var, 0, Kc, rep, rep_stride, out_stride, mix_sample, mix_mean, mix_var));
      if (L.mean_W) return conv_mean_add(ctx, L, X, n_mod, 0, Kc, rep, out_stride, mix_mean, mix_sample);
      return DCGP_OK;
    }
    if (ride_head) return ctx_fail(ctx, DCGP_ERR_ARG, "conv layer: the step was planned to carry the head's rows in a launch the layer does not take");
  }
  int chunk_rows = rows;
  if (!keep_state)
    while (chunk_rows > 1 && (long)Mp * col_ld((long)chunk_rows * P) * 8 >= (1L << 31)) chunk_rows = (chunk_rows + 1) / 2;
  const bool chunked = chunk_rows < rows;
  if (chunked && !(phase & 2)) return DCGP_OK;
  const long ldc = col_ld((long)chunk_rows * P);
  double* B = (double*)ws_get(ctx, pfx + "Kuf", (size_t)Mp * ldc * sizeof(double));
  if (!B) return DCGP_ERR_ALLOC;
  if ((phase & 1 || chunked) && Mp > L.M) HIP_TRY(ctx, hipMemsetAsync(B + (size_t)L.M * ldc, 0, (size_t)(Mp - L.M) * ldc * sizeof(double), ctx->stream));
  for (int r0 = 0; r0 < rows; r0 += chunk_rows) {
    const int nr = rows - r0 < chunk_rows ? rows - r0 : chunk_rows;
    const long kc = (long)nr * P;
    PatchRbfArgs a;
    a.X = X; a.N = nr; a.n_mod = n_mod; a.n0 = r0;
    a.H = L.v.H; a.W = L.v.W; a.C = L.v.C; a.f = L.v.f; a.s = L.v.s; a.Ho = L.v.Ho; a.Wo = L.v.Wo; a.P = P; a.L = L.v.L;
    a.ZT = L.ZT; a.zn = L.zn; a.M = L.M; a.Mp = Mp; a.Lp = L.Lp;
    a.bk = L.base();
    a.out = B; a.sM = ldc; a.sN = P; a.sP = 1;
    a.share_cu = phase == 1;
    a.patch_scale = L.in_scale;
    if ((phase & 1) || chunked) {
      bool done = false;
      if (a.bk.type == 0 && !L.in_scale) {
        HeadUnitsArgs h;
        h.X = X; h.n_mod = n_mod; h.N = nr; h.n0 = r0;
        h.H = L.v.H; h.W = L.v.W; h.C = L.v.C; h.f = L.v.f; h.s = L.v.s; h.Wo = L.v.Wo; h.P = P; h.L = L.v.L; h.Lq = L.Lz;
        h.ZS = L.ZS; h.M = L.M; h.Mp = Mp;
        h.csq = sqrt(1.4426950408889634074) / L.ls; h.log2var = log2(L.variance);
        h.kuf = B; h.sM = ldc; h.sN = P; h.sP = 1;
        h.share_cu = phase == 1;
        h.upw_force = (int)ctx->opt.kuf_upw;
        h.stream_k = (int)ctx->opt.kuf_stream;
        h.wpg_force = (int)ctx->opt.kuf_wpg;
        h.split_force = (int)ctx->opt.kuf_split;
        h.occ_force = (int)ctx->opt.sweep_occ;
        h.share_kb = (int)ctx->opt.share_kb;
        h.no_rep = (int)ctx->opt.kuf_no_rep;
        h.timer = L.v.L > 64 ? "kuf_long" : "kuf";
        head_units_plan(&h);
        if (head_units_ok(h)) { DCGP_TRY(head_units(ctx, h)); done = true; }
      }
      if (!done) DCGP_TRY(patch_rbf(ctx, a, "kuf"));
    }
    if (!(phase & 2)) return DCGP_OK;
    if (factor_done && r0 == 0) HIP_TRY(ctx, hipStreamWaitEvent(ctx->stream, factor_done, 0));
    CondScratch sc;
    DCGP_TRY(cond_core(ctx, L.g, B, ldc, (int)kc, L.white, L.has_qsqrt, pfx.c_str(), &sc, r0 == 0 ? prep_done : nullptr));
    FinalizeArgs fa;
    fa.s1p = sc.s1p; fa.nrb1 = sc.nrb1; fa.s2p = sc.s2p; fa.nrb3 = sc.nrb3; fa.mu = sc.mu; fa.ldk = ldc;
    fa.Kc = (int)kc; fa.R = L.R; fa.knn_scalar = L.variance; fa.col0 = (long)r0 * P;
    fa.rep = rep; fa.rep_stride = rep_stride; fa.z = z; fa.seed = seed; fa.stream_id = stream_id; fa.jitter = jitter;
    fa.out_sample = out_sample; fa.out_mean = out_mean; fa.out_var = out_var;
    if (rmap) fa.rmap = *rmap;
    if (L.identity_mean) {
      fa.X = X; fa.idm = 1; fa.H = L.v.H; fa.W = L.v.W; fa.C = L.v.C; fa.f = L.v.f; fa.s = L.v.s; fa.Wo = L.v.Wo; fa.P = P;
      fa.n_mod = n_mod;
    }
    DCGP_TRY(finalize_layer(ctx, fa));
    if (L.mix_W)
      DCGP_TRY(mix_forward(ctx, L.mix_W, L.R, L.Rout, out_sample, out_mean, out_var, (long)r0 * P, kc, rep, rep_stride, out_stride, mix_sample, mix_mean, mix_var));
    if (L.mean_W) DCGP_TRY(conv_mean_add(ctx, L, X, n_mod, (long)r0 * P, kc, rep, out_stride, mix_mean, mix_sample));
  }
  return DCGP_OK;
}

static inline int head_forward(dcgp_ctx* ctx, LayerState& L, const double* X, int rows, int n_mod, double* kd, double* out_mean,
                 double* out_var, const std::string& pfx, hipEvent_t factor_done = nullptr,
                               hipEvent_t prep_done = nullptr, int sweep_mode = 0, bool* early_done = nullptr,
                               bool keep_k = false, KlOffer* kl = nullptr, int kzx_done = 0) {
  const int Mp = L.Mp;
  const long ldb = col_ld(rows);
  if (sweep_mode != 2) L.kfull_ready = false;
  if (sweep_mode != 1) L.a1h_ready = false;
  double* a1_out = nullptr;
  if (keep_k && sweep_mode != 1 && !ctx->opt.grad_no_keep_k && head_cond_fused_ok(L.g) && !ctx->opt.head_unfused) {
    a1_out = (double*)ws_get(ctx, pfx + "g_A1h", (size_t)Mp * ldb * sizeof(double));
    if (!a1_out) return DCGP_ERR_ALLOC;
  }
  double* B = (double*)ws_get(ctx, pfx + "Kzx", (size_t)Mp * ldb * sizeof(double));
  if (!B) return DCGP_ERR_ALLOC;
  if (sweep_mode != 2 && Mp > L.M) HIP_TRY(ctx, hipMemsetAsync(B + (size_t)L.M * ldb, 0, (size_t)(Mp - L.M) * ldb * sizeof(double), ctx->stream));
  PatchRbfArgs a;
  a.X = X; a.N = rows; a.n_mod = n_mod;
  a.H = L.v.H; a.W = L.v.W; a.C = L.v.C; a.f = L.v.f; a.s = L.v.s; a.Ho = L.v.Ho; a.Wo = L.v.Wo; a.P = L.v.P; a.L = L.v.L;
  a.ZT = L.ZT; a.zn = L.zn; a.M = L.M; a.Mp = Mp; a.Lp = L.Lp;
  a.bk = L.base();
  a.out = B; a.sM = ldb; a.sN = 1; a.sP = 0;
  a.w = L.w; a.scale = 1.0 / (double)L.v.P; a.reduce = 1;
  a.in_scale = L.in_scale;
  const bool unfused = ctx->opt.head_unfused != 0;
  if (L.kernel_type == 0 && a.bk.type == 0 && !L.in_scale) {
    HeadUnitsArgs h = head_sweep_shape(ctx, L, X, rows, n_mod, B, ldb);
    h.share_cu = factor_done != nullptr;
    if (keep_k && !ctx->opt.grad_no_keep_k && L.v.L >= 64) {
      const long ldf = col_ld((long)rows * L.v.P);
      h.kfull = (double*)ws_get(ctx, pfx + "g_Kfull", (size_t)Mp * ldf * sizeof(double));
      if (!h.kfull) return DCGP_ERR_ALLOC;
      h.kf_sM = ldf; h.kf_sN = L.v.P;
    }
    head_units_plan(&h);
    if (h.kfull && !head_units_ok(h)) { h.kfull = nullptr; head_units_plan(&h); }
    if (head_units_ok(h)) {
      if (sweep_mode != 2) L.kfull_ready = h.kfull != nullptr;
      h.kd = (double*)ws_get(ctx, "kdiag_partial", (size_t)rows * h.n_kd * sizeof(double));
      if (!h.kd) return DCGP_ERR_ALLOC;
      if (kzx_done) {
        if (sweep_mode != 0 || h.kfull || h.nseg < 2 || h.seg[0].kind != 0)
          return ctx_fail(ctx, DCGP_ERR_ARG, "head: its Kzx rows were run by the layer kernel, but the sweep is not the one that was planned");
        if (kzx_done > rows) return ctx_fail(ctx, DCGP_ERR_ARG, "head: more Kzx rows done than the head has");
        const int gone = h.seg[0].wpi * kzx_done;
        for (int q = 1; q < h.nseg; ++q) h.seg[q].wg0 -= gone;
        h.n_wgs -= gone;
        if (kzx_done < rows) h.seg[0].img0 = kzx_done;
        else {
          for (int q = 1; q < h.nseg; ++q) h.seg[q - 1] = h.seg[q];
          --h.nseg;
        }
      }
      if (sweep_mode != 2) DCGP_TRY(head_units(ctx, h));
      if (sweep_mode == 1) {
        if (early_done) *early_done = true;
        return DCGP_OK;
      }
      const double kd_scale = 1.0 / ((double)L.v.P * (double)L.v.P);
      if (prep_done) HIP_TRY(ctx, hipStreamWaitEvent(ctx->stream, prep_done, 0));
      else if (factor_done) HIP_TRY(ctx, hipStreamWaitEvent(ctx->stream, factor_done, 0));
      if (head_cond_fused_ok(L.g) && !unfused) {
        L.a1h_ready = a1_out != nullptr;
        return head_cond_fused(ctx, L.g, B, ldb, rows, L.has_qsqrt, h.kd, out_mean, out_var, h.n_kd, kd_scale, a1_out, ldb, kl);
      }
      DCGP_TRY(kdiag_reduce(ctx, h.kd, h.n_kd, rows, kd_scale, kd));
      CondScratch sc;
      DCGP_TRY(cond_core(ctx, L.g, B, ldb, rows, L.white, L.has_qsqrt, pfx.c_str(), &sc, nullptr, true));
      FinalizeArgs fa;
      fa.s1p = sc.s1p; fa.nrb1 = sc.nrb1; fa.s2p = sc.s2p; fa.nrb3 = sc.nrb3; fa.mu = sc.mu; fa.ldk = ldb;
      fa.Kc = rows; fa.R = L.R; fa.knn_vec = kd;
      fa.out_mean = out_mean; fa.out_var = out_var;
      return finalize_layer(ctx, fa);
    }
  }
  if (kzx_done) return ctx_fail(ctx, DCGP_ERR_ARG, "head: its Kzx rows were run by the layer kernel, but the head does not take the unit sweep");
  if (sweep_mode == 1) return DCGP_OK;
  if (L.kernel_type == 0 && a.bk.type == 0 && head_cond_fused_ok(L.g) && !unfused) {
    const double* kdp = nullptr; int kd_n = 1; double kd_scale = 1.0;
    DCGP_TRY(head_sweep(ctx, a, L.w, &kdp, &kd_n, &kd_scale));
    if (prep_done) HIP_TRY(ctx, hipStreamWaitEvent(ctx->stream, prep_done, 0));
    else if (factor_done) HIP_TRY(ctx, hipStreamWaitEvent(ctx->stream, factor_done, 0));
    L.a1h_ready = a1_out != nullptr;
    return head_cond_fused(ctx, L.g, B, ldb, rows, L.has_qsqrt, kdp, out_mean, out_var, kd_n, kd_scale, a1_out, ldb, kl);
  }
  hipStream_t main_s = ctx->stream;
  const bool kd_on_side = !ctx->no_side;
  if (kd_on_side) {
    HIP_TRY(ctx, hipEventRecord(ctx->ev_aux, main_s));
    HIP_TRY(ctx, hipStreamWaitEvent(ctx->stream_aux, ctx->ev_aux, 0));
    ctx->stream = ctx->stream_aux;
  }
  int rc;
  if (L.kernel_type == 0) {
    rc = head_kdiag(ctx, X, rows, n_mod, L.v.H, L.v.W, L.v.C, L.v.f, L.v.s, L.base(), L.w, kd);
  } else {
    rc = additive_kdiag_async(ctx, rows, L.v.P, L.variance, L.w, kd);
  }
  if (kd_on_side) {
    if (rc == DCGP_OK && hipEventRecord(ctx->ev_aux2, ctx->stream_aux) != hipSuccess) rc = DCGP_ERR_HIP;
    ctx->stream = main_s;
  }
  DCGP_TRY(rc);
  DCGP_TRY(patch_rbf(ctx, a, "head_kzx"));
  if (factor_done) HIP_TRY(ctx, hipStreamWaitEvent(ctx->stream, factor_done, 0));
  if (head_cond_fused_ok(L.g) && !unfused) {
    if (prep_done) HIP_TRY(ctx, hipStreamWaitEvent(ctx->stream, prep_done, 0));
    if (!ctx->no_side) HIP_TRY(ctx, hipStreamWaitEvent(ctx->stream, ctx->ev_aux2, 0));
    return head_cond_fused(ctx, L.g, B, ldb, rows, L.has_qsqrt, kd, out_mean, out_var, 1, 1.0, nullptr, 0, kl);
  }
  CondScratch sc;
  DCGP_TRY(cond_core(ctx, L.g, B, ldb, rows, L.white, L.has_qsqrt, pfx.c_str(), &sc, prep_done, true));
  if (!ctx->no_side) HIP_TRY(ctx, hipStreamWaitEvent(ctx->stream, ctx->ev_aux2, 0));
  FinalizeArgs fa;
  fa.s1p = sc.s1p; fa.nrb1 = sc.nrb1; fa.s2p = sc.s2p; fa.nrb3 = sc.nrb3; fa.mu = sc.mu; fa.ldk = ldb;
  fa.Kc = rows; fa.R = L.R; fa.knn_vec = kd;
  fa.out_mean = out_mean; fa.out_var = out_var;
  return finalize_layer(ctx, fa);
}
```

### deepcgp_amd/csrc/model.hip

```cpp
#include <chrono>
#include <cstdlib>
#include <cstring>
#include <memory>

#include "model_state.h"
#include "tail_dev.h"

namespace {

int g_model_counter = 0;

int build_groups(dcgp_model* m, int bank) {
  if (m->groups_built[bank]) return DCGP_OK;
  auto& groups = m->groups[bank];
  for (auto& gr : groups) gr.release();
  groups.clear();
  auto add = [&](int Mp, double* K, double* Linv, double* LinvT, const ChainRhs& r) {
    FactorGroup* g = nullptr;
    for (auto& gr : groups)
      if (gr.Mp == Mp) g = &gr;
    if (!g) { groups.emplace_back(); g = &groups.back(); g->Mp = Mp; }
    g->K.push_back(K); g->Linv.push_back(Linv); g->LinvT.push_back(LinvT); g->rhs.push_back(r);
    if (r.Lq || r.qmu) { g->ride = true; g->max_R = r.R > g->max_R ? r.R : g->max_R; }
  };
// ... 24 lines not shown
  m->events_ok = true;
  return DCGP_OK;
}

int ensure(dcgp_ctx* ctx, double** p, size_t* cap, size_t n) {
  if (*cap >= n && *p) return DCGP_OK;
  if (*p) { hipDeviceSynchronize(); dev_free(ctx, *p); *p = nullptr; }
  if (dev_alloc(ctx, (void**)p, (n ? n : 2) * sizeof(double), "model_scratch") != hipSuccess) return ctx_fail(ctx, DCGP_ERR_ALLOC, "model: allocation failed");
  *cap = n;
  return DCGP_OK;
}

int ensure_out(dcgp_model* m, int li, int rows, int width) {
  auto& o = m->outs[li];
  size_t n = (size_t)rows * width;
  if (o.cap < n) {
    hipDeviceSynchronize();
    dev_free(m->ctx, o.sample); dev_free(m->ctx, o.mean); dev_free(m->ctx, o.var);
    o.sample = o.mean = o.var = nullptr;
    if (dev_alloc(m->ctx, (void**)&o.sample, n * sizeof(double), "out_sample") != hipSuccess ||
        dev_alloc(m->ctx, (void**)&o.mean, n * sizeof(double), "out_mean") != hipSuccess ||
        dev_alloc(m->ctx, (void**)&o.var, n * sizeof(double), "out_var") != hipSuccess)
      return ctx_fail(m->ctx, DCGP_ERR_ALLOC, "model: output allocation failed");
    o.cap = n;
  }
  o.rows = rows; o.width = width;
  return DCGP_OK;
}

__global__ void combine_kernel(double* __restrict__ scal, ElboFinish fin) {
  if (threadIdx.x == 0 && blockIdx.x == 0) elbo_assemble(scal, fin, scal[0]);
}

int read_info(dcgp_model* m, int* info_host) {
  dcgp_ctx* ctx = m->ctx;
  int bad = 0;
  for (auto& gr : m->groups[m->bank]) {
    std::vector<int> h(gr.K.size());
    HIP_TRY(ctx, hipMemcpyAsync(h.data(), gr.d_info, h.size() * sizeof(int), hipMemcpyDeviceToHost, ctx->stream));
    HIP_TRY(ctx, hipStreamSynchronize(ctx->stream));
    for (int v : h)
      if (v && !bad) bad = v;
  }
  if (info_host) *info_host = bad;
  if (bad) return ctx_fail(ctx, DCGP_ERR_NOT_PD, "Cholesky: matrix not positive definite at column %d", bad);
  return DCGP_OK;
}
int finish_inference(dcgp_model* m, int* info_host) {
  HIP_TRY(m->ctx, hipStreamSynchronize(m->ctx->stream));
  return read_info(m, info_host);
}

struct StreamGuard {
  dcgp_ctx* ctx; hipStream_t saved;
  explicit StreamGuard(dcgp_ctx* c) : ctx(c), saved(c->stream) {}
  ~StreamGuard() { ctx->stream = saved; ctx->ws_tag.clear(); }
};

int fill_finish(dcgp_model* model, double scale, int slot, ElboFinish* fin) {
  const int nl = (int)model->layers.size();
  fin->nl = nl; fin->scale = scale;
  for (int l = 0; l < nl; ++l) { fin->M[l] = model->layers[l]->M; fin->R[l] = model->layers[l]->R; fin->white[l] = model->layers[l]->white; }
  DCGP_TRY(fill_status(model, &fin->st));
  fin->host_out = model->h_ring_dev + 8 * slot;
  fin->host_seq = (double)(model->enq_seq + 1);
  return DCGP_OK;
}


enum class PrepPlace { OnChain, SplitChainFirst, SplitSweepFirst };
enum class ForkMark { BehindFirstLayer, BehindChain };

struct StepPlan {
  bool reuse = false;
  int bank = 0, rows0 = 0;
  hipStream_t main_s = nullptr, chain_s = nullptr, kl_s = nullptr;
  bool first_one_launch = true;
  PrepPlace prep = PrepPlace::OnChain;
  bool early_sweep = false;
  bool defer = false;
  ChainMode chain;
  ForkMark mark = ForkMark::BehindFirstLayer;
  int ride_layer = -1, ride_rows = 0;
  bool chain_beside() const { return chain_s != main_s; }
};
struct StepIn { const double* X; int N, S; const double* const* zs; uint64_t seed; int dedup; bool need_kl; };
std::string model_pfx(const dcgp_model* m) { return "m" + std::to_string(m->id) + "_"; }

StepPlan plan_step(const dcgp_model* m, int N, int S, int dedup, bool need_kl, bool pipelined) {
  const dcgp_ctx* ctx = m->ctx;
  const LayerState& L0 = *m->layers[0];
  StepPlan p;
  p.reuse = !pipelined && !m->grad_follows && (!m->keep_state || m->data_grad) && m->chain_version == m->param_version && m->chain_with_kl == need_kl &&
            m->factor_reuse >= (need_kl ? 2 : 1) && !ctx->opt.no_factor_reuse;
  p.bank = p.reuse ? m->bank : m->bank ^ 1;
  const bool part = pipelined && ctx->stream_m && !ctx->no_side;
  p.main_s = part ? ctx->stream_m : ctx->stream;
  p.kl_s = ctx->no_side ? p.main_s : (part ? ctx->stream2_m : (pipelined ? (p.bank ? ctx->stream2b : ctx->stream2) : ctx->stream2));
  p.rows0 = dedup ? N : S * N;
  p.first_one_launch = first_layer_one_launch(ctx, L0, p.rows0);
  p.chain_s = p.reuse ? p.main_s : ((pipelined || !p.first_one_launch) ? p.kl_s : p.main_s);
  p.early_sweep = p.chain_beside() && !p.first_one_launch && !ctx->opt.no_early_sweep;
  if (p.early_sweep && !pipelined && !ctx->opt.prep_on_chain) p.prep = L0.is_head ? PrepPlace::SplitSweepFirst : PrepPlace::SplitChainFirst;
  bool one_group = true;
  for (auto& l : m->layers) one_group = one_group && l->Mp == L0.Mp;
  p.defer = one_group && need_kl && !m->keep_state;
  p.chain = ChainMode{!p.chain_beside() && !pipelined, p.first_one_launch};
  p.mark = (long)p.rows0 * L0.v.P >= 8192 ? ForkMark::BehindFirstLayer : ForkMark::BehindChain;
  const int nl = (int)m->layers.size();
  if (nl >= 2 && m->layers[nl - 1]->is_head && !m->layers[nl - 2]->is_head && m->pad[nl - 1] == 0 && !m->layers[nl - 2]->mean_W && !m->layers[nl - 2]->mix_W) {
    const int li = nl - 2;
    const LayerState& Lc = *m->layers[li];
    const LayerState& Lh = *m->layers[nl - 1];
    const bool expand = dedup && li == 0;
    const int rows_in = li == 0 ? p.rows0 : S * N, rows_out = S * N;
    ConvFusedArgs fa = conv_fused_shape(Lc, rows_in);
    fa.n_mod = li == 0 ? N : rows_in; fa.rep = expand ? S : 1;
    HeadUnitsArgs h = head_sweep_shape(ctx, Lh, nullptr, rows_out, rows_out, nullptr, col_ld(rows_out));
    head_units_plan(&h);
    const bool form = head_sweep_rides_form(ctx, Lh, h) && !(m->keep_state && m->grad_follows);
    if (li > 0 || p.first_one_launch)
      p.ride_rows = conv_fused_rides_head(ctx, fa, m->keep_state, form, h.HWC, (long)head_units_lds(h), h.nfm, pipelined, p.chain_beside() && !p.reuse);
    if (p.ride_rows > 0) p.ride_layer = li;
  }
  return p;
}

struct ChainScope {
  dcgp_ctx* ctx; const StepPlan& p; bool ok = false;
  ChainScope(dcgp_model* m, const StepPlan& plan) : ctx(m->ctx), p(plan) { ctx->stream = p.chain_s; ctx->ws_tag = "~m" + std::to_string(m->id) + "b" + std::to_string(p.bank); }
  ~ChainScope() {
    ctx->stream = p.main_s; ctx->ws_tag.clear();
    if (!ok) { hipStreamSynchronize(p.kl_s); hipStreamSynchronize(p.chain_s); }
  }
};

int check_padding(dcgp_model* m) {
  if (!m->any_pad || m->pad_ok) return DCGP_OK;
  dcgp_ctx* ctx = m->ctx;
  const int nl = (int)m->layers.size();
  for (int li = 0; li < nl && li < 8; ++li) {
    const int p = m->pad[li];
    if (p == 0) continue;
    const LayerState& L = *m->layers[li];
    if (p < 0) return ctx_fail(ctx, DCGP_ERR_ARG, "padding: layer %d has a negative padding (%d)", li, p);
    if (L.is_head && L.in_scale)
      return ctx_fail(ctx, DCGP_ERR_ARG, "padding: layer %d is a dense head, only conv layers and patch heads take padding", li);
    if (L.v.H - 2 * p < 1 || L.v.W - 2 * p < 1)
      return ctx_fail(ctx, DCGP_ERR_ARG, "padding: layer %d was added as %d x %d, smaller than its border of %d (add the layer with the padded size)", li,
                      L.v.H, L.v.W, p);
    if (li == 0) continue;
    const LayerState& B = *m->layers[li - 1];
    if (B.is_head || B.v.Ho + 2 * p != L.v.H || B.v.Wo + 2 * p != L.v.W || B.Rout != L.v.C)
      return ctx_fail(ctx, DCGP_ERR_ARG, "padding: layer %d takes %d x %d x %d, layer %d produces %d x %d x %d and the padding is %d", li, L.v.H, L.v.W, L.v.C,
                      li - 1, B.v.Ho, B.v.Wo, B.Rout, p);
  }
  m->pad_ok = true;
  return DCGP_OK;
}

int pad_input(dcgp_model* m, hipStream_t stream, int li, int bank, const double* src, long rows, const double** out) {
  dcgp_ctx* ctx = m->ctx;
  const LayerState& L = *m->layers[li];
  const int p = m->pad[li];
  const std::string name = "m" + std::to_string(m->id) + "_" + std::to_string(li) + "_Xpad" + (li == 0 ? "_b" + std::to_string(bank) : std::string());
  double* dst = (double*)ws_get(ctx, name, (size_t)rows * L.v.H * L.v.W * L.v.C * sizeof(double));
  if (!dst) return DCGP_ERR_ALLOC;
  DCGP_TRY(pad_images(ctx, stream, src, rows, L.v.H - 2 * p, L.v.W - 2 * p, L.v.C, p, dst));
  m->pad_in[li] = dst;
  *out = dst;
  return DCGP_OK;
}

int run_layer(dcgp_model* m, const StepPlan& p, const StepIn& in, int li, const double* F, int rows, int n_mod, int phase, bool* head_swept, KlOffer* kl,
              int* out_rows_p) {
  dcgp_ctx* ctx = m->ctx;
  LayerState& L = *m->layers[li];
  const std::string pfx = model_pfx(m) + std::to_string(li) + "_";
  const double* z = in.zs ? in.zs[li] : nullptr;
  hipEvent_t fdone = (li == 0 && p.chain_beside()) ? m->ev_factor[p.bank] : nullptr;
  hipEvent_t pdone = p.chain_beside() ? m->ev_prep[p.bank][li] : nullptr;
  if (!L.is_head) {
    const int width = L.v.P * L.Rout, lat_width = L.v.P * L.R;
    const bool expand = in.dedup && li == 0;
    const int out_rows = expand ? in.S * in.N : rows;
    DCGP_TRY(ensure_out(m, li, out_rows, width));
    if (L.mix_W) DCGP_TRY(L.ensure_latent((size_t)out_rows * lat_width));
    auto& o = m->outs[li];
    RngMap rm;
    const bool sharded = m->shard_global > 0;
    if (sharded && (m->shard_global != in.N || m->shard_lo != 0)) { rm.W = lat_width; rm.Nl = in.N; rm.Ng = m->shard_global; rm.lo = m->shard_lo; }
    HeadUnitsArgs ride;
    if (li == p.ride_layer && (phase & 2)) {
      LayerState& Lh = *m->layers[li + 1];
      const long ldh = col_ld(out_rows);
      double* B = (double*)ws_get(ctx, model_pfx(m) + std::to_string(li + 1) + "_" + "Kzx", (size_t)Lh.Mp * ldh * sizeof(double));
      if (!B) return DCGP_ERR_ALLOC;
      ride = head_sweep_shape(ctx, Lh, o.sample, out_rows, out_rows, B, ldh);
      head_units_plan(&ride);
    }
    DCGP_TRY(conv_forward(ctx, L, F, rows, n_mod, expand ? in.S : 1, (long)in.N * lat_width, z, in.seed, (uint32_t)(li + 1 + (sharded ? 0 : 64 * ctx->rank)),
                          m->jitter, o.sample, m->keep_outputs ? o.mean : nullptr, m->keep_outputs ? o.var : nullptr, pfx,
                          fdone, pdone, phase, m->keep_state, &rm, li == 0 ? (int)p.first_one_launch : -1,
                          (li == p.ride_layer && (phase & 2)) ? &ride : nullptr, p.ride_rows));
    *out_rows_p = out_rows;
    return DCGP_OK;
  }
  DCGP_TRY(ensure_out(m, li, rows, L.R));
  auto& o = m->outs[li];
  DCGP_TRY(ensure(ctx, &m->d_kd, &m->kd_cap, (size_t)rows));
  DCGP_TRY(head_forward(ctx, L, F, rows, n_mod, m->d_kd, o.mean, o.var, pfx, fdone, pdone,
                        phase == 1 ? 1 : (phase == 2 && *head_swept ? 2 : 0), phase == 1 ? head_swept : nullptr,
                        m->keep_state && m->grad_follows, kl, (p.ride_layer == li - 1 && p.ride_layer >= 0) ? p.ride_rows : 0));
  *out_rows_p = rows;
  if (phase != 1 && m->keep_outputs) {
    size_t n = (size_t)rows * L.R;
    if (z) {
      DCGP_TRY(reparam_async(ctx, o.mean, o.var, z, n, m->jitter, o.sample));
    } else {
      HIP_TRY(ctx, hipMemcpyAsync(o.sample, o.mean, n * sizeof(double), hipMemcpyDeviceToDevice, ctx->stream));
    }
  }
  return DCGP_OK;
}

int enqueue_chain(dcgp_model* m, const StepPlan& p, const StepIn& in, bool* early0, bool* head_swept) {
  dcgp_ctx* ctx = m->ctx;
  const int nl = (int)m->layers.size(), bank = p.bank;
  const bool beside = p.chain_beside();
  if (beside && m->done_valid[bank]) HIP_TRY(ctx, hipStreamWaitEvent(p.chain_s, m->done_ev[bank], 0));
  else if (beside && ctx->ev_last_valid) HIP_TRY(ctx, hipStreamWaitEvent(p.chain_s, ctx->ev_last, 0));
  PrepArgs pa;
  pa.nl = nl;
  for (int li = 0; li < nl; ++li) pa.l[li] = m->layers[li]->prep_args(m->jitter);
  if (p.prep == PrepPlace::OnChain) {
    DCGP_TRY(prepare_all(ctx, pa));
    if (beside && !p.first_one_launch) HIP_TRY(ctx, hipEventRecord(m->ev_sweep[bank], p.chain_s));
  } else {
    if (p.prep == PrepPlace::SplitChainFirst) DCGP_TRY(prepare_all(ctx, pa, ~kPrepSweepTasks));
    ctx->stream = p.main_s;
    DCGP_TRY(prepare_all(ctx, pa, kPrepSweepTasks));
    ctx->stream = p.chain_s;
  }
  if (p.early_sweep) {
    ctx->stream = p.main_s;
    if (p.prep == PrepPlace::OnChain) HIP_TRY(ctx, hipStreamWaitEvent(p.main_s, m->ev_sweep[bank], 0));
    int out_rows = 0;
    DCGP_TRY(run_layer(m, p, in, 0, in.X, p.rows0, in.N, 1, head_swept, nullptr, &out_rows));
    *early0 = true;
    ctx->stream = p.chain_s;
  }
  if (p.prep == PrepPlace::SplitSweepFirst) DCGP_TRY(prepare_all(ctx, pa, ~kPrepSweepTasks));
  for (auto& gr : m->groups[bank]) DCGP_TRY(gr.run(ctx, p.defer, p.chain));
  if (beside) HIP_TRY(ctx, hipEventRecord(m->ev_factor[bank], p.chain_s));
  bool made[8] = {}, rode[8] = {};
  for (int li = 0; li < nl; ++li) {
    LayerState& L = *m->layers[li];
    bool live_sums = false, prior_sums = false;
    for (auto& gr : m->groups[bank]) {
      if (!gr.rode) continue;
      for (size_t i = 0; i < gr.K.size(); ++i) {
        if (gr.K[i] == L.g.K && (gr.rhs[i].Lq || gr.rhs[i].qmu)) { rode[li] = true; live_sums = gr.rhs[i].Lq != nullptr; }
        if (L.g.Kp && gr.K[i] == L.g.Kp && gr.rhs[i].Lq) prior_sums = true;
      }
    }
    if (!(made[li] = rode[li])) continue;
    L.g.klp_valid = live_sums; L.g.klpp_valid = prior_sums;
    L.g.kl_ns = chain_rhs_slots(L.Mp); L.g.kl_nsa = (L.Mp + 31) / 32;
  }
  GpMats* gs[8]; int wh[8]; bool hq[8];
  for (int li = 0; li < nl; ++li) { gs[li] = &m->layers[li]->g; wh[li] = m->layers[li]->white; hq[li] = m->layers[li]->has_qsqrt; }
  DCGP_TRY(prep_solve_all(ctx, gs, wh, hq, nl, made, rode));
  for (int li = 0; li < nl; ++li) {
    if (!made[li]) DCGP_TRY(cond_prep(ctx, m->layers[li]->g, m->layers[li]->white, m->layers[li]->has_qsqrt));
    if (beside) HIP_TRY(ctx, hipEventRecord(m->ev_prep[bank][li], p.chain_s));
  }
  return DCGP_OK;
}

int place_kl(dcgp_model* m, const StepPlan& p, bool need_kl, double* scal, bool* join) {
  dcgp_ctx* ctx = m->ctx;
  const int nl = (int)m->layers.size(), bank = p.bank;
  bool in_tail = need_kl && !ctx->opt.kl_side;
  for (int li = 0; li < nl && in_tail; ++li) {
    const LayerState& L = *m->layers[li];
    in_tail = !L.white && L.has_qsqrt && L.g.klp_valid && (!L.g.Kp || L.g.klpp_valid);
  }
  m->kl_in_tail[bank] = in_tail;
  if (in_tail) {
    KlTail& kt = m->kl_tail[bank];
    kt.nl = nl;
    const auto it = p.defer ? ctx->ws.find("chol_Lout" + ctx->ws_tag) : ctx->ws.end();
    const double* lout = it != ctx->ws.end() ? (const double*)it->second.first : nullptr;
    for (int li = 0; li < nl; ++li) {
      const LayerState& L = *m->layers[li];
      KlTailLayer& q = kt.l[li];
// ... 855 lines not shown
```

### deepcgp_amd/device.py

```python
import ctypes as C
import os
import re

import numpy as np

_HERE = os.path.dirname(os.path.abspath(__file__))
LIB_PATH = os.environ.get("DCGP_LIB", os.path.join(_HERE, "libdcgp.so"))
HEADER_PATH = os.path.join(os.path.dirname(_HERE), "include", "dcgp.h")

DCGP_OK, ERR_ARG, ERR_HIP, ERR_NOT_PD, ERR_RCCL, ERR_ALLOC = 0, -1, -2, -3, -4, -5
OBJECTIVE_DENSITY, OBJECTIVE_ELBO, INPUT_GRAD_DEDUP = 0, 1, 0x100


class LibraryMissing(RuntimeError):
    """libdcgp.so is not built (run `python -c "import __graft_entry__ as g; g.build()"`)."""


class DcgpError(RuntimeError):
    def __init__(self, code, msg):
        super().__init__("libdcgp error %d: %s" % (code, msg))
        self.code = code


class NotPositiveDefinite(DcgpError, np.linalg.LinAlgError):
# ... 57 lines not shown
    "dcgp_quad_varexp": [_vp, _i, _vp, _vp, _vp, _vp, _i, _i, _vp],
    "dcgp_quad_predict": [_vp, _i, _vp, _vp, _vp, _i, _i, _vp, _vp],
    "dcgp_quad_logdensity": [_vp, _i, _vp, _vp, _vp, _vp, _i, _i, _vp],
    "dcgp_quad_grad_seeds": [_vp, _i, _vp, _vp, _vp, _vp, _i, _i, _d, _vp, _vp, _vp],
    "dcgp_reparam": [_vp, _vp, _vp, _vp, _sz, _d, _vp],
    "dcgp_model_create": [_vp, _i, _d, C.POINTER(_vp)],
    "dcgp_model_destroy": [_vp],
    "dcgp_model_add_conv_layer": [_vp, _i, _i, _i, _i, _i, _i, _i, _i, _i, _d, _d, _vp, _vp, _vp, _vp],
    "dcgp_model_set_head": [_vp, _i, _i, _i, _i, _i, _i, _i, _i, _i, _d, _d, _vp, _vp, _vp, _vp],
    "dcgp_model_set_keep_outputs": [_vp, _i],
    "dcgp_model_set_param": [_vp, _i, C.c_char_p, _vp, _sz],
    "dcgp_elbo_forward": [_vp, _vp, _vp, _i, _d, C.POINTER(_vp), _u64, _i, _dp, _ip],
    "dcgp_elbo_forward_enqueue": [_vp, _vp, _vp, _i, _d, C.POINTER(_vp), _u64, _i, C.POINTER(_u64)],
    "dcgp_elbo_forward_collect": [_vp, _u64, _dp, _ip],
    "dcgp_model_propagate": [_vp, _vp, _i, _i, C.POINTER(_vp), _u64, _vp, _vp, _ip],
    "dcgp_elbo_grad": [_vp, _vp, _vp, _i, _d, C.POINTER(_vp), _u64, _i, C.POINTER(_d), _ip],
    "dcgp_model_get_grad": [_vp, _i, C.c_char_p, _vp, C.c_size_t],
    "dcgp_model_adam_step": [_vp, _d, _d, _d, _d, _i],
    "dcgp_model_train_step_adam": [_vp, _vp, _vp, _i, _d, C.POINTER(_vp), _u64, _i, _d, _d, _d, _d, _i, C.POINTER(_d), _ip],
    "dcgp_model_set_dataset": [_vp, _vp, _vp, C.c_long, _i],
    "dcgp_model_train_run_adam": [_vp, _vp, _i, _i, _d, _vp, _u64, _i, _d, _d, _d, _vp, _ip, _ip],
    "dcgp_model_set_augmentation": [_vp, _i, _i, _i, _i, _i],
    "dcgp_augment_images": [_vp, _vp, _i, _i, _i, _i, _i, _i, _u64, _vp],
    "dcgp_model_set_eval_views": [_vp, _i, _i, _i, _i, _vp],
    "dcgp_view_images": [_vp, _vp, _i, _i, _i, _i, _i, _vp, _vp],
    "dcgp_model_get_param": [_vp, _i, C.c_char_p, _vp, C.c_size_t],
    "dcgp_model_set_grad_shards": [_vp, _i],
    "dcgp_model_set_shard": [_vp, _i, _i],
    "dcgp_model_set_input_padding": [_vp, _i, _i],
    "dcgp_model_set_mean_filter": [_vp, _i, _vp, _i],
    "dcgp_debug_conv_mean_time": [_vp, _i, _i, _i, _i, _i, _i, _i, _i, _i, _dp],
    "dcgp_model_set_mixing": [_vp, _i, _vp, _i, _i],
    "dcgp_mix_forward": [_vp, _vp, _i, _i, _vp, _vp, _vp, C.c_long, C.c_long, _i, C.c_long, C.c_long, _vp, _vp, _vp],
    "dcgp_mix_backward": [_vp, _vp, _i, _i, _vp, _vp, C.c_long, _vp, _vp],
    "dcgp_debug_mix_time": [_vp, _i, _i, C.c_long, _i, _dp],
    "dcgp_model_grad_block": [_vp, _i, C.POINTER(_vp), C.POINTER(C.c_size_t)],
    "dcgp_model_sgd_step": [_vp, _d],
    "dcgp_model_get_adam_state": [_vp, _i, C.c_char_p, _vp, _vp, C.c_size_t],
    "dcgp_model_set_adam_state": [_vp, _i, C.c_char_p, _vp, _vp, C.c_size_t],
    "dcgp_model_get_adam_t": [_vp, _ip],
    "dcgp_model_set_adam_t": [_vp, _i],
    "dcgp_model_set_grad_clip": [_vp, _d],
    "dcgp_model_grad_norms": [_vp, _vp, _i, _ip],
    "dcgp_model_set_grad_exchange": [_vp, _i],
    "dcgp_model_debug_sharded_adam": [_vp, _i, _d, _d, _d, _d, _i],
    "dcgp_shard_range": [C.c_long, _i, _i, C.POINTER(C.c_long), C.POINTER(C.c_long), C.POINTER(C.c_long)],
    "dcgp_model_set_trainable": [_vp, _i, C.c_char_p, _i],
    "dcgp_model_set_factor_reuse": [_vp, _i],
    "dcgp_model_chain_skips": [_vp, C.POINTER(_u64)],
    "dcgp_model_factor_groups": [_vp, _i, _ip, _ip, _ip, _ip],
    "dcgp_model_natgrad_step": [_vp, _d, _ip],
    "dcgp_model_predict_y": [_vp, _vp, _i, _i, C.POINTER(_vp), _u64, _vp, _vp, _ip],
    "dcgp_model_predict_density": [_vp, _vp, _vp, _i, _i, C.POINTER(_vp), _u64, _vp, _ip],
    "dcgp_model_input_grad": [_vp, _vp, _vp, _i, _i, C.POINTER(_vp), _u64, _i, _vp, _vp, _ip],
    "dcgp_model_input_grad_f64y": [_vp, _vp, _vp, _i, _i, C.POINTER(_vp), _u64, _i, _vp, _vp, _ip],
    "dcgp_model_evaluate": [_vp, _vp, _vp, _i, _i, _i, C.POINTER(_vp), _u64, _vp, _vp, _dp, _ip],
    "dcgp_model_layer_output": [_vp, _i, _vp, _vp, _vp, _ip, _ip],
    "dcgp_model_set_likelihood": [_vp, _i, _d],
    "dcgp_model_set_likelihood_nodes": [_vp, _vp, _i],
    "dcgp_model_set_likelihood_params": [_vp, _i, _vp, _i],
    "dcgp_elbo_forward_f64y": [_vp, _vp, _vp, _i, _d, C.POINTER(_vp), _u64, _i, _dp, _ip],
    "dcgp_elbo_forward_enqueue_f64y": [_vp, _vp, _vp, _i, _d, C.POINTER(_vp), _u64, _i, C.POINTER(_u64)],
    "dcgp_elbo_grad_f64y": [_vp, _vp, _vp, _i, _d, C.POINTER(_vp), _u64, _i, C.POINTER(_d), _ip],
    "dcgp_model_train_step_adam_f64y": [_vp, _vp, _vp, _i, _d, C.POINTER(_vp), _u64, _i, _d, _d, _d, _d, _i, C.POINTER(_d), _ip],
    "dcgp_model_predict_mean_var": [_vp, _vp, _i, _i, C.POINTER(_vp), _u64, _vp, _vp, _ip],
    "dcgp_model_predict_density_f64y": [_vp, _vp, _vp, _i, _i, C.POINTER(_vp), _u64, _vp, _ip],
    "dcgp_model_evaluate_f64y": [_vp, _vp, _vp, _i, _i, _i, C.POINTER(_vp), _u64, _vp, _vp, _dp, _ip],
    "dcgp_model_evaluate_uncertainty": [_vp, _vp, _vp, _i, _i, _i, C.POINTER(_vp), _u64, _i, _vp, _vp, _vp, _vp, _vp, _vp, _vp, _vp, _dp, _ip],
    "dcgp_model_evaluate_uncertainty_f64y": [_vp, _vp, _vp, _i, _i, _i, C.POINTER(_vp), _u64, _i, _vp, _vp, _vp, _vp, _vp, _vp, _vp, _vp, _dp,
                                             _ip],
    "dcgp_convkernel_patch_mean": [_vp, _vp, _i, _i, _i, _i, _i, _i, _vp, _i, _d, _d, _vp, _vp, _i, _vp],
    "dcgp_model_patch_evidence": [_vp, _vp, _i, _i, C.POINTER(_vp), _u64, _vp, _vp, _ip],
    "dcgp_gemm_strided": [_vp, _vp, C.c_long, C.c_long, C.c_long, _vp, C.c_long, C.c_long, C.c_long, _vp, C.c_long, C.c_long,
                          _i, _i, _i, _i, _d, _i, _vp, C.c_long, C.c_long, _vp, C.c_long, C.c_long, _i],
    "dcgp_gemm_strided_ex": [_vp, _vp, C.c_long, C.c_long, C.c_long, _vp, C.c_long, C.c_long, C.c_long, _vp, C.c_long, C.c_long,
                             _i, _i, _i, _i, _d, _i, _vp, C.c_long, _vp, C.c_long, C.c_long, _i],
    "dcgp_kmeans": [_vp, _vp, C.c_long, _i, _i, _vp, _i, _d, _vp, _ip],
    "dcgp_debug_set_fused_trace": [_vp, _vp],
    "dcgp_debug_fused_plan": [_vp, _vp],
    "dcgp_debug_plan_layer_launch": [_vp, _i, _vp, _i],
    "dcgp_debug_plan_gemm": [_vp, _i, _vp, _i],
    "dcgp_debug_head_ride": [_vp, _vp],
    "dcgp_debug_plan_head_ride": [_vp, _i, _vp, _i, C.c_longlong, _vp, _i],
    "dcgp_debug_comm_gate": [_vp, _i, _ip],
    "dcgp_debug_mfma_f64_rate": [_vp, _dp],
    "dcgp_debug_store_rate": [_vp, _i, _i, _i, _dp],
    "dcgp_debug_set_sweep_trace": [_vp, _vp, C.c_long, C.c_char_p],
    "dcgp_comm_unique_id": [C.c_char_p],
    "dcgp_comm_init_rank": [_vp, _i, _i, C.c_char_p],
    "dcgp_comm_destroy": [_vp],
    "dcgp_comm_count": [_vp, _ip],
    "dcgp_allreduce_sum_f64": [_vp, _vp, _i],
}
_RESTYPE = {"dcgp_last_error": C.c_char_p}

_lib = None


def declared_symbols():
    with open(HEADER_PATH) as fh:
        return sorted(set(re.findall(r"\b(dcgp_[a-z0-9_]+)\s*\(", fh.read())))


def lib():
    global _lib
    if _lib is None:
        if not os.path.exists(LIB_PATH):
            raise LibraryMissing("%s not found -- build it with __graft_entry__.build() "
                                 "(make -C deepcgp_amd/csrc); there is no CPU fallback" % LIB_PATH)
        L = C.CDLL(LIB_PATH)
        for name, args in _SIGS.items():
            fn = getattr(L, name)
            fn.argtypes = args
            fn.restype = _RESTYPE.get(name, C.c_int)
        _lib = L
    return _lib


def device_count():
    n = C.c_int(0)
    lib().dcgp_device_count(C.byref(n))
    return n.value


class DeviceArray:

    def __init__(self, ctx, shape, dtype=np.float64):
        self.ctx = ctx
        self.shape = tuple(int(s) for s in shape)
        self.dtype = np.dtype(dtype)
        self.nbytes = int(np.prod(self.shape, dtype=np.int64)) * self.dtype.itemsize
        p = _vp()
        ctx._check(lib().dcgp_malloc(ctx.handle, max(self.nbytes, 16), C.byref(p)))
        self.ptr = p.value

    @property
    def size(self):
        return int(np.prod(self.shape, dtype=np.int64))

    def numpy(self):
        out = np.empty(self.shape, self.dtype)
        if self.nbytes:
            self.ctx._check(lib().dcgp_d2h(self.ctx.handle, out.ctypes.data, self.ptr, self.nbytes))
        return out

    def set(self, host):
        host = np.ascontiguousarray(host, self.dtype)
        assert host.size == self.size, (host.shape, self.shape)
        if self.nbytes:
            self.ctx._check(lib().dcgp_h2d(self.ctx.handle, self.ptr, host.ctypes.data, self.nbytes))
        return self

    def free(self):
        if getattr(self, "ptr", None) and self.ctx.handle:
            lib().dcgp_free(self.ctx.handle, self.ptr)
        self.ptr = None

    def __del__(self):
        try:
            self.free()
        except Exception:
            pass


class Context:

# ... 153 lines not shown
```

### include/dcgp.h

```cpp
#ifndef DCGP_H
#define DCGP_H

#include <stddef.h>
#include <stdint.h>

#ifdef __cplusplus
extern "C" {
#endif

#define DCGP_OK 0
#define DCGP_ERR_ARG (-1)
#define DCGP_ERR_HIP (-2)
#define DCGP_ERR_NOT_PD (-3)
#define DCGP_ERR_RCCL (-4)
#define DCGP_ERR_ALLOC (-5)

typedef struct dcgp_ctx dcgp_ctx;
typedef struct dcgp_model dcgp_model;

int dcgp_ctx_create(int device, dcgp_ctx** out);
int dcgp_ctx_destroy(dcgp_ctx* ctx);
const char* dcgp_last_error(dcgp_ctx* ctx);
int dcgp_device_count(int* count);
int dcgp_malloc(dcgp_ctx* ctx, size_t bytes, void** dptr);
// ... 156 lines not shown
                         double* out_fmean, double* out_fvar, int* info_host);
int dcgp_model_predict_y(dcgp_model* model, const double* X, int N, int S,
                         const double* const* z_per_layer_host, uint64_t seed,
                         double* out_p, double* out_p_mean, int* info_host);
int dcgp_model_predict_density(dcgp_model* model, const double* X, const int32_t* y, int N, int S,
                               const double* const* z_per_layer, uint64_t seed, double* out_logdens, int* info_host);
#define DCGP_OBJECTIVE_DENSITY 0
#define DCGP_OBJECTIVE_ELBO 1
#define DCGP_INPUT_GRAD_DEDUP 0x100
int dcgp_model_input_grad(dcgp_model* model, const double* X, const int32_t* y, int N, int S,
                          const double* const* z_per_layer, uint64_t seed, int objective,
                          double* out_value, double* out_dX, int* info_host);
int dcgp_model_evaluate(dcgp_model* model, const double* X, const int32_t* y, int N_total, int batch, int S,
                        const double* const* z_per_layer, uint64_t seed, double* out_logdens, double* out_p_mean,
                        double* out_host, int* info_host);

int dcgp_model_set_likelihood(dcgp_model* model, int kind, double variance);
int dcgp_model_set_likelihood_nodes(dcgp_model* model, const double* nodes_host, int Q);
int dcgp_model_set_likelihood_params(dcgp_model* model, int kind, const double* params_host, int n);
int dcgp_elbo_forward_f64y(dcgp_model* model, const double* X, const double* y, int N, double scale,
                           const double* const* z_per_layer_host, uint64_t seed, int dedup_layer0, double* out_host,
                           int* info_host);
int dcgp_elbo_forward_enqueue_f64y(dcgp_model* model, const double* X, const double* y, int N, double scale,
                                   const double* const* z_per_layer_host, uint64_t seed, int dedup_layer0, uint64_t* ticket);
int dcgp_elbo_grad_f64y(dcgp_model* model, const double* X, const double* y, int N, double scale,
                        const double* const* z_per_layer_host, uint64_t seed, int dedup_layer0, double* out_host,
                        int* info_host);
int dcgp_model_train_step_adam_f64y(dcgp_model* model, const double* X, const double* y, int N, double scale,
                                    const double* const* z_per_layer_host, uint64_t seed, int dedup_layer0, double lr, double beta1,
                                    double beta2, double eps, int t, double* out_host, int* info_host);
int dcgp_model_predict_mean_var(dcgp_model* model, const double* X, int N, int S,
                                const double* const* z_per_layer_host, uint64_t seed,
                                double* out_mean, double* out_var, int* info_host);
int dcgp_model_patch_evidence(dcgp_model* model, const double* X, int N, int S, const double* const* z_per_layer, uint64_t seed,
                              double* out_c, double* out_fmean, int* info_host);
int dcgp_model_predict_density_f64y(dcgp_model* model, const double* X, const double* y, int N, int S,
                                    const double* const* z_per_layer, uint64_t seed, double* out_logdens, int* info_host);
int dcgp_model_input_grad_f64y(dcgp_model* model, const double* X, const double* y, int N, int S,
                               const double* const* z_per_layer, uint64_t seed, int objective,
                               double* out_value, double* out_dX, int* info_host);
int dcgp_model_evaluate_f64y(dcgp_model* model, const double* X, const double* y, int N_total, int batch, int S,
                             const double* const* z_per_layer, uint64_t seed, double* out_logdens, double* out_y_mean,
                             double* out_host, int* info_host);
int dcgp_model_evaluate_uncertainty(dcgp_model* model, const double* X, const int32_t* y, int N_total, int batch, int S,
                                    const double* const* z_per_layer, uint64_t seed, int bins, double* out_logdens, double* out_p_mean,
                                    double* out_pred_entropy, double* out_exp_entropy, double* out_mutual_info, double* out_confidence,
                                    int32_t* out_prediction, double* out_table, double* out_host, int* info_host);
int dcgp_model_evaluate_uncertainty_f64y(dcgp_model* model, const double* X, const double* y, int N_total, int batch, int S,
                                         const double* const* z_per_layer, uint64_t seed, int bins, double* out_logdens, double* out_p_mean,
                                         double* out_pred_entropy, double* out_exp_entropy, double* out_mutual_info,
                                         double* out_confidence, int32_t* out_prediction, double* out_table, double* out_host,
                                         int* info_host);
int dcgp_model_set_factor_reuse(dcgp_model* model, int mode);
int dcgp_model_chain_skips(dcgp_model* model, uint64_t* out);
int dcgp_model_factor_groups(dcgp_model* model, int cap, int* count_out, int* Mp_out, int* matrices_out, int* riding_out);
int dcgp_model_layer_output(dcgp_model* model, int layer, double* out_sample, double* out_mean,
                            double* out_var, int* rows, int* width);

int dcgp_gemm_strided(dcgp_ctx* ctx, const double* A, long a_rs, long a_cs, long a_bs, const double* B, long b_rs,
                      long b_cs, long b_bs, double* C, long c_rs, long c_bs, int M, int N, int K, int batch,
                      double alpha, int accumulate, const double* colscale, long cs_s, long cs_bs,
                      const double* kscale, long ks_s, long ks_bs, int flags);
int dcgp_gemm_strided_ex(dcgp_ctx* ctx, const double* A, long a_rs, long a_cs, long a_bs, const double* B, long b_rs,
                         long b_cs, long b_bs, double* C, long c_rs, long c_bs, int M, int N, int K, int batch,
                         double alpha, int accumulate, const double* sub_v, long sv_bs, const double* sub_x, long sx_rs,
                         long sx_bs, int flags);

int dcgp_kmeans(dcgp_ctx* ctx, const double* X, long n, int d, int k, const int32_t* init_rows_host, int max_iter,
                double tol, double* centers, int* iters_out);

int dcgp_comm_unique_id(unsigned char* out_128bytes);
int dcgp_comm_init_rank(dcgp_ctx* ctx, int nranks, int rank, const unsigned char* id_128bytes);
int dcgp_comm_destroy(dcgp_ctx* ctx);
int dcgp_comm_count(dcgp_ctx* ctx, int* out_ranks);
int dcgp_allreduce_sum_f64(dcgp_ctx* ctx, double* buf_dev, int n);

int dcgp_debug_comm_gate(dcgp_ctx* ctx, int closed, int* main_idle_out);
int dcgp_debug_set_fused_trace(dcgp_ctx* ctx, long long* buf_dev);
int dcgp_debug_fused_plan(dcgp_ctx* ctx, int* out4);
int dcgp_debug_plan_layer_launch(const long long* query, int n_query, long long* plan, int n_plan);
int dcgp_debug_plan_gemm(const long long* query, int n_query, long long* plan, int n_plan);
int dcgp_debug_head_ride(dcgp_ctx* ctx, long long* out2);
int dcgp_debug_plan_head_ride(const long long* query, int n_query, const long long* ride, int n_ride, long long row, long long* out, int n_out);
int dcgp_debug_mfma_f64_rate(dcgp_ctx* ctx, double* tflops_out);
int dcgp_debug_store_rate(dcgp_ctx* ctx, int N, int P, int M, double* gbs_out);
int dcgp_debug_set_sweep_trace(dcgp_ctx* ctx, long long* buf_dev, long n_workgroups, const char* family );
int dcgp_debug_conv_mean_time(dcgp_ctx* ctx, int H, int W, int C, int f, int stride, int R, int rows, int rep, int iters, double* out_us);

int dcgp_debug_mix_time(dcgp_ctx* ctx, int G, int R, long Kc, int iters, double* out_us);

#ifdef __cplusplus
}
#endif
#endif
```

Before: 1402 ELBO steps/s.

## Carry the head's full unit sweep as tail items inside the fused conv layer launch

Extends the head-ride mechanism so the persistent fused conv kernel also runs the remaining head Kzx rows, split into sub-parts across waves, plus the Kdiag chunks as extra tail work items after the layer strips. When the tail rides, the head skips its separate head_units launch. A cost model (DealSim) picks the number of parts and enables the tail only when it predicts the makespan shrinks. This adds a new kernel instantiation, more per-item branching and flag waits, and tighter coupling between the layer and head plans.

New measurement: 1428 ELBO steps/s, median of 6. 1.9% higher.

```diff
diff --git a/deepcgp_amd/csrc/common.h b/deepcgp_amd/csrc/common.h
--- a/deepcgp_amd/csrc/common.h
+++ b/deepcgp_amd/csrc/common.h
@@ -35,6 +35,7 @@
   long fused_parts = -1;
   long fused_rep_share = -1;
   long head_ride = -1;
+  long head_ride_tail = -1;
   long fused_wgs = 0;
   long fused_stagger = -1;
   long kl_side = 0;
@@ -99,6 +100,7 @@
   hipEvent_t ev_aux = nullptr, ev_aux2 = nullptr;
   std::string err;
   int last_head_rows = 0; long head_ride_launches = 0;
+  int last_tail_kd = 0, last_tail_sub = 0, last_tail_parts = 0; long head_sweeps_skipped = 0;
   unsigned fused_head_epoch = 0;
   unsigned fused_pre_epoch = 0;
   std::string ws_tag;
diff --git a/deepcgp_amd/csrc/conv_fused.hip b/deepcgp_amd/csrc/conv_fused.hip
--- a/deepcgp_amd/csrc/conv_fused.hip
+++ b/deepcgp_amd/csrc/conv_fused.hip
@@ -71,7 +71,7 @@
     strip_next = __builtin_amdgcn_readfirstlane(tk[0]);
     __syncthreads();
   }
-  const int first_limit = HEAD ? a.n_items + a.head_n : (a.pre_n > 0 ? a.n_items : 0x7fffffff);
+  const int first_limit = HEAD ? a.n_items + a.head_n + a.tail_n : (a.pre_n > 0 ? a.n_items : 0x7fffffff);
   for (int it = 0; strip_next < first_limit; ++it) {
   int tid = threadIdx.x;
   asm volatile("" : "+s"(ap), "+v"(tid));
@@ -79,7 +79,19 @@
   if constexpr (HEAD) {
     if (strip_next >= a.n_items) {
       int* tk = reinterpret_cast<int*>(smem + a.lds_main + a.lds_img + BN);
-      const int row = strip_next - a.n_items;
+      const int hit = strip_next - a.n_items;
+      int row = hit, kz_lo = 0, kz_n = -1, kd = 0;
+      if (HEAD > 1 && hit >= a.head_n) {
+        const int t = hit - a.head_n, n_sub = a.tail_n - a.head_n;
+        if (t >= n_sub) { row = t - n_sub; kz_n = 0; kd = 1; }
+        else {
+          const int j = t, rr = j / a.tail_parts, part = j - rr * a.tail_parts;
+          row = a.head_n + rr;
+          kz_lo = part * a.tail_upp;
+          kz_n = min(a.tail_upp, a.head.nfm - kz_lo);
+          kd = part == a.tail_parts - 1 ? 1 : 0;
+        }
+      }
       if (tid == 0) {
         const int s_hi = (row * a.P + a.P - 1) / BN;
         int ok = 1;
@@ -94,9 +106,25 @@
       }
       __syncthreads();
       if (tk[1]) {
-        head_units_dev::head_units_body<0, 50, 0, NT, true>(ap->head, row);
+        if constexpr (HEAD > 1) {
+        const int wv = __builtin_amdgcn_readfirstlane(tid >> 6);
+        int sg = 0, u = 0x7fff;
+        if (kz_n < 0) u = (wv + row) & (W - 1);
+        else if (wv < kz_n) u = kz_lo + wv;
+        else if (kd) {
+          sg = 1;
+          for (int q = 2; q < 6; ++q)
+            if (q < a.head.nseg && row >= a.head.seg[q].img0) sg = q;
+          u = wv - kz_n;
+        }
+        head_units_dev::head_units_body<0, 50, 0, NT, true, true>(ap->head, row, sg, u);
+        } else {
+          head_units_dev::head_units_body<0, 50, 0, NT, true>(ap->head, row);
+        }
       } else {
-        for (int m = tid; m < a.head.kzx_rows; m += NT) a.head.kzx[(long)m * a.head.ldk + row] = __builtin_nan("");
+        const int m_lo = kz_n < 0 ? 0 : 16 * kz_lo, m_hi = kz_n < 0 ? a.head.kzx_rows : min(16 * (kz_lo + kz_n), a.head.kzx_rows);
+        for (int m = m_lo + tid; m < m_hi; m += NT) a.head.kzx[(long)m * a.head.ldk + row] = __builtin_nan("");
+        if (HEAD > 1 && kd && tid < a.head.n_kd) a.head.kd[(long)row * a.head.n_kd + tid] = __builtin_nan("");
       }
       if (tid == 0) tk[0] = atomicAdd(a.dyn, 1);
       __syncthreads();
@@ -750,9 +778,9 @@
 }
 template <int I>
 int launch_fused(dcgp_ctx* ctx, const ConvFusedArgs& a, const Plan& p) {
-  if (a.head_n > 0) {
+  if (a.head_n > 0 || a.tail_parts > 0) {
     if constexpr (I == 0) {
-      if (!p.patch_rows && a.bk.type == 0) return launch_instance<0, 0, 1>(ctx, a, p);
+      if (!p.patch_rows && a.bk.type == 0) return a.tail_parts > 0 ? launch_instance<0, 0, 2>(ctx, a, p) : launch_instance<0, 0, 1>(ctx, a, p);
     }
     return ctx_fail(ctx, DCGP_ERR_ARG, "conv_fused: head rows on a launch that cannot carry them (shape %d)", I);
   }
@@ -827,6 +855,37 @@
     for (long st = lo; st <= hi; ++st) last = std::max(last, fused_plan::ride_sample_item(p, st));
   }
   const long long flat[8] = {rd.ok, rd.why, rd.n_rows, rd.first_item, rd.ok ? rd.first_item + row : -1, lo, hi, last};
+  memcpy(out, flat, sizeof flat);
+  return DCGP_OK;
+}
+
+extern "C" int dcgp_debug_head_tail(dcgp_ctx* ctx, long long* out4) {
+  if (!ctx || !out4) return DCGP_ERR_ARG;
+  out4[0] = ctx->last_tail_kd; out4[1] = ctx->last_tail_sub; out4[2] = ctx->last_tail_parts; out4[3] = ctx->head_sweeps_skipped;
+  return DCGP_OK;
+}
+
+extern "C" int dcgp_debug_plan_head_tail(const long long* query, int n_query, const long long* ride, int n_ride, const long long* tail, int n_tail, long long item,
+                                         long long* out, int n_out) {
+  if (!query || !ride || !tail || !out || n_query != Query::kFields || n_ride != fused_plan::RideQuery::kFields || n_tail != fused_plan::TailQuery::kFields || n_out != 14)
+    return DCGP_ERR_ARG;
+  Query q;
+  std::apply([&](auto&... f) { ((f = (long)*query++), ...); }, Query::fields(q));
+  fused_plan::RideQuery r;
+  r.next_is_head = ride[0]; r.head_form = ride[1]; r.head_HWC = ride[2]; r.head_lds = ride[3]; r.head_nfm = ride[4]; r.in_flight = ride[5]; r.chain_beside = ride[6];
+  r.head_ride = ride[7];
+  fused_plan::TailQuery t;
+  t.head_ride_tail = tail[0]; t.n_kd = tail[1];
+  const Plan p = fused_plan::plan_layer_launch(q);
+  const fused_plan::Tail tl = fused_plan::plan_head_tail(q, p, r, t);
+  fused_plan::TailItem ti{-1, 0, 0, 0};
+  long lo = 0, hi = -1, last = -1;
+  if (tl.ok && item >= 0 && item < tl.n_items) {
+    ti = fused_plan::tail_item(tl, r.head_nfm, item);
+    fused_plan::ride_row_strips(ti.row, q.P, kShapes[p.shape].FN * 16, &lo, &hi);
+    for (long st = lo; st <= hi; ++st) last = std::max(last, fused_plan::ride_sample_item(p, st));
+  }
+  const long long flat[14] = {tl.ok, tl.why, tl.n_rows, tl.parts, tl.upp, tl.first_item, tl.n_items, ti.row, ti.kz_lo, ti.kz_hi, ti.kd, lo, hi, last};
   memcpy(out, flat, sizeof flat);
   return DCGP_OK;
 }
@@ -863,6 +922,23 @@
   return fused_plan::plan_head_ride(q, fused_plan::plan_layer_launch(q), r).n_rows;
 }
 
+int conv_fused_head_tail(const dcgp_ctx* ctx, const ConvFusedArgs& a, bool keeps_state, bool head_form, long head_HWC, long head_lds, long head_nfm, long head_n_kd,
+                         bool in_flight, bool chain_beside, int* n_rows) {
+  *n_rows = 0;
+  if (ctx->opt.no_fused_layer) return 0;
+  Query q = fused_query(ctx, a);
+  q.keeps_state = keeps_state;
+  fused_plan::RideQuery r;
+  r.next_is_head = 1; r.head_form = head_form; r.head_HWC = head_HWC; r.head_lds = head_lds; r.head_nfm = head_nfm; r.in_flight = in_flight;
+  r.chain_beside = chain_beside; r.head_ride = ctx->opt.head_ride;
+  fused_plan::TailQuery t;
+  t.head_ride_tail = ctx->opt.head_ride_tail; t.n_kd = head_n_kd;
+  const fused_plan::Tail tail = fused_plan::plan_head_tail_memo(q, r, t);
+  if (!tail.ok) return 0;
+  *n_rows = tail.n_rows;
+  return tail.parts;
+}
+
 int conv_fused(dcgp_ctx* ctx, const ConvFusedArgs& a_in) {
   if (a_in.Kc <= 0) return DCGP_OK;
   const Plan p = fused_plan::plan_layer_launch(fused_query(ctx, a_in));
@@ -879,7 +955,43 @@
   }
   if (p.cu_slots) DCGP_TRY(ws_zeroed(ctx, "fused_cu_slots", 1024 * sizeof(int), &a.cu_slots));
   ctx->last_head_rows = 0;
-  if (a.head_n > 0) {
+  ctx->last_tail_kd = ctx->last_tail_sub = ctx->last_tail_parts = 0;
+  a.tail_n = a.tail_upp = 0;
+  if (a.tail_parts > 0) {
+    fused_plan::RideQuery rq;
+    rq.next_is_head = 1; rq.head_form = 1; rq.head_HWC = a.head.HWC; rq.head_lds = (long)head_units_lds(a.head); rq.head_nfm = a.head.nfm;
+    rq.head_ride = ctx->opt.head_ride;
+    fused_plan::TailQuery tq;
+    tq.head_ride_tail = ctx->opt.head_ride_tail; tq.n_kd = a.head.n_kd;
+    const fused_plan::Tail tail = fused_plan::plan_head_tail_memo(fused_query(ctx, a_in), rq, tq);
+    if (!tail.ok || tail.n_rows != a.head_n || tail.parts != a.tail_parts || a.head.X != a.out_sample || a.head.N != a_in.Kc / a_in.P || a.head.n_mod < a.head.N ||
+        a.head.n0 != 0 || !a.head.kzx || !a.head.kd || a.head.kuf || a.head.kfull || a.head.trace)
+      return ctx_fail(ctx, DCGP_ERR_ARG, "conv_fused: the launch cannot carry the head's sweep (reason %d)", tail.why);
+    HuSeg segs[6];
+    int ns = 1, next_img = 0;
+    for (int g = 0; g < a.head.nseg; ++g) {
+      const HuSeg& s = a.head.seg[g];
+      if (s.kind != 1) continue;
+      if (ns >= 6 || s.img0 != next_img || s.upw != 1 || s.C < 1 || s.C > a.head.n_kd || s.T < 1)
+        return ctx_fail(ctx, DCGP_ERR_ARG, "conv_fused: the head's Kdiag segments are not the plan the tail items were written for");
+      segs[ns] = s;
+      next_img = g + 1 < a.head.nseg ? a.head.seg[g + 1].img0 : a.head.N;
+      ++ns;
+    }
+    if (ns < 2) return ctx_fail(ctx, DCGP_ERR_ARG, "conv_fused: the head's sweep has no Kdiag chunks to carry");
+    segs[0] = HuSeg{};
+    a.head.nseg = ns;
+    for (int g = 0; g < ns; ++g) a.head.seg[g] = segs[g];
+    a.head.n_wgs = a.head_n + tail.n_items; a.head.upw = 1;
+    a.tail_n = tail.n_items; a.tail_upp = tail.upp;
+    bool cleared = false;
+    DCGP_TRY(ws_zeroed(ctx, "fused_head_flag", (size_t)p.n_strips * sizeof(unsigned), &a.head_flag, ctx->fused_head_epoch == 0xffffffffu, &cleared));
+    if (cleared) ctx->fused_head_epoch = 0;
+    a.head_epoch = ++ctx->fused_head_epoch;
+    ctx->last_head_rows = a.head_n;
+    ctx->last_tail_kd = a.head_n; ctx->last_tail_sub = tail.n_items - a.head_n; ctx->last_tail_parts = tail.parts;
+    ++ctx->head_ride_launches;
+  } else if (a.head_n > 0) {
     fused_plan::RideQuery rq;
     rq.next_is_head = 1; rq.head_form = 1; rq.head_HWC = a.head.HWC; rq.head_lds = (long)head_units_lds(a.head); rq.head_nfm = a.head.nfm;
     rq.head_ride = ctx->opt.head_ride;
diff --git a/deepcgp_amd/csrc/ctx.hip b/deepcgp_amd/csrc/ctx.hip
--- a/deepcgp_amd/csrc/ctx.hip
+++ b/deepcgp_amd/csrc/ctx.hip
@@ -28,7 +28,7 @@
     {"kuf_wpg", &DcgpOptions::kuf_wpg}, {"kuf_split", &DcgpOptions::kuf_split}, {"head_tail", &DcgpOptions::head_tail},
     {"sweep_occ", &DcgpOptions::sweep_occ}, {"share_kb", &DcgpOptions::share_kb}, {"head_upw", &DcgpOptions::head_upw}, {"no_syrk", &DcgpOptions::no_syrk}, {"grad_dz_main", &DcgpOptions::grad_dz_main},
     {"fused_persist", &DcgpOptions::fused_persist}, {"fused_stagger", &DcgpOptions::fused_stagger}, {"fused_pre", &DcgpOptions::fused_pre}, {"fused_parts", &DcgpOptions::fused_parts},
-    {"fused_rep_share", &DcgpOptions::fused_rep_share}, {"fused_wgs", &DcgpOptions::fused_wgs}, {"head_ride", &DcgpOptions::head_ride},
+    {"fused_rep_share", &DcgpOptions::fused_rep_share}, {"fused_wgs", &DcgpOptions::fused_wgs}, {"head_ride", &DcgpOptions::head_ride}, {"head_ride_tail", &DcgpOptions::head_ride_tail},
     {"fused_abl", &DcgpOptions::fused_abl}, {"rb_mixed", &DcgpOptions::rb_mixed},
 };
 }
diff --git a/deepcgp_amd/csrc/fused_plan.h b/deepcgp_amd/csrc/fused_plan.h
--- a/deepcgp_amd/csrc/fused_plan.h
+++ b/deepcgp_amd/csrc/fused_plan.h
@@ -75,6 +75,7 @@
     else if (kind == kPrologueOnly) ready_[(size_t)slot] = run(kCostPrologue + kCostHandOver, 0.0);
     else run(kCostHandOver + outputs + kCostEpilogue, ready_[(size_t)slot]);
   }
+  void give_cost(double cost) { run(cost, 0.0); }
   double makespan() const { return end_; }
   std::vector<double> free_times() const {
     std::vector<double> out;
@@ -289,9 +290,8 @@
   int first_item = 0;
 };
 constexpr double kCostHeadRow = 3.0;
-inline long ride_room(const Query& q, const Plan& p) {
-  const long S = p.persist, strips = p.n_strips, R = q.R;
-  DealSim d(S, R, p.pre_n);
+inline void deal_plan_items(DealSim& d, const Query& q, const Plan& p) {
+  const long strips = p.n_strips, R = q.R;
   if (p.pre_D > 0) {
     for (long i = 0; i < strips; ++i) {
       if (i < p.pre_D) d.give(kLeaving, i);
@@ -306,6 +306,10 @@
   } else {
     for (long i = 0; i < strips; ++i) d.give(kWhole);
   }
+}
+inline long ride_room(const Query& q, const Plan& p) {
+  DealSim d(p.persist, q.R, p.pre_n);
+  deal_plan_items(d, q, p);
   long room = 0;
   for (double t : d.free_times()) room += (long)((d.makespan() - t + kEps) / kCostHeadRow);
   return room;
@@ -338,4 +342,100 @@
   return strip;
 }
 
-}
+struct TailQuery {
+  long head_ride_tail = -1;
+  long n_kd = 0;
+  static constexpr int kFields = 2;
+};
+enum TailWhy { kTailRides = 0, kTailOff, kTailNoRide, kTailGeometry, kTailFewWorkgroups, kTailNoGain };
+struct Tail {
+  int ok = 0, why = kTailOff;
+  int n_rows = 0;
+  int parts = 1, upp = 0;
+  int first_item = 0;
+  int n_items = 0;
+  double units_sweep = 0.0, units_tail = 0.0;
+};
+struct TailItem { int row, kz_lo, kz_hi, kd; };
+inline TailItem tail_item(const Tail& t, long nfm, long i) {
+  const long n_sub = t.n_items - t.n_rows;
+  if (i >= n_sub) return TailItem{(int)(i - n_sub), 0, 0, 1};
+  const long row = t.n_rows + i / t.parts, part = i % t.parts;
+  return TailItem{(int)row, (int)(part * t.upp), (int)std::min<long>(nfm, (part + 1) * t.upp), part == t.parts - 1 ? 1 : 0};
+}
+constexpr double kCostTailKd = 0.9, kCostTailHalf = 1.4, kCostTailQuarter = 0.95;
+constexpr double kCostSweepKzx = 3.3, kCostSweepKd = 2.0;
+constexpr double kTailMargin = 0.5;
+inline bool tail_parts_ok(long parts, long nfm, long n_kd, long waves) {
+  if (parts < 1 || parts > nfm) return false;
+  const long upp = (nfm + parts - 1) / parts;
+  return (parts - 1) * upp < nfm && (nfm - (parts - 1) * upp) + n_kd <= waves;
+}
+inline double tail_units(const Query& q, const Plan& p, long rows, long n_rows, long parts) {
+  DealSim d(p.persist, q.R, p.pre_n);
+  deal_plan_items(d, q, p);
+  for (long i = 0; i < n_rows; ++i) d.give_cost(kCostHeadRow);
+  if (parts <= 0) return d.makespan();
+  const double part = parts >= 4 ? kCostTailQuarter : (parts >= 2 ? kCostTailHalf : kCostHeadRow);
+  for (long i = 0; i < (rows - n_rows) * parts; ++i) d.give_cost(part);
+  for (long i = 0; i < n_rows; ++i) d.give_cost(kCostTailKd);
+  return d.makespan();
+}
+inline Tail plan_head_tail(const Query& q, const Plan& p, const RideQuery& r, const TailQuery& t) {
+  Tail out;
+  auto no = [&](int why) { out.ok = 0; out.why = why; return out; };
+  if (t.head_ride_tail == 0) return no(kTailOff);
+  const Ride ride = plan_head_ride(q, p, r);
+  if (!ride.ok && ride.why != kRideNoRoom) return no(kTailNoRide);
+  const long waves = kShapes[0].NT / 64, nfm = r.head_nfm, rows = q.Kc / q.P;
+  if (t.n_kd < 1 || t.n_kd > waves) return no(kTailGeometry);
+  const bool chosen = t.head_ride_tail < 0;
+  if (chosen && p.persist != (q.n_cus > 0 ? q.n_cus : 256)) return no(kTailFewWorkgroups);
+  long parts = 0;
+  if (t.head_ride_tail > 1) {
+    if (!tail_parts_ok(t.head_ride_tail, nfm, t.n_kd, waves)) return no(kTailGeometry);
+    parts = t.head_ride_tail;
+  }
+  const long n_rows = ride.ok ? ride.n_rows : 0;
+  if (chosen) {
+    out.units_sweep = tail_units(q, p, rows, n_rows, 0) + (n_rows < rows ? kCostSweepKzx : kCostSweepKd);
+    double best = out.units_sweep - kTailMargin;
+    long best_parts = 0;
+    for (long s : {2L, 4L, 1L}) {
+      if (!tail_parts_ok(s, nfm, t.n_kd, waves)) continue;
+      const double u = tail_units(q, p, rows, n_rows, s);
+      if (u < best - kEps) { best = u; best_parts = s; }
+    }
+    if (!best_parts) return no(kTailNoGain);
+    parts = best_parts;
+    out.units_tail = best;
+  } else if (!parts) {
+    for (long s : {1L, 4L, 2L})
+      if (tail_parts_ok(s, nfm, t.n_kd, waves)) parts = s;
+    if (!parts) return no(kTailGeometry);
+  }
+  out.ok = 1; out.why = kTailRides;
+  out.n_rows = (int)n_rows;
+  out.parts = (int)parts; out.upp = (int)((nfm + parts - 1) / parts);
+  out.first_item = p.n_items + (int)n_rows;
+  out.n_items = (int)(n_rows + (rows - n_rows) * parts);
+  return out;
+}
+inline Tail plan_head_tail_memo(const Query& q, const RideQuery& r, const TailQuery& t) {
+  if (t.head_ride_tail == 0) return Tail{};
+  static std::mutex mu;
+  static std::map<std::tuple<Query, std::tuple<long, long, long, long, long, long, long, long, long, long>>, Tail> memo;
+  const auto key = std::make_tuple(q, std::make_tuple(r.next_is_head, r.head_form, r.head_HWC, r.head_lds, r.head_nfm, r.in_flight, r.chain_beside, r.head_ride,
+                                                      t.head_ride_tail, t.n_kd));
+  {
+    std::lock_guard<std::mutex> lock(mu);
+    const auto it = memo.find(key);
+    if (it != memo.end()) return it->second;
+  }
+  const Tail out = plan_head_tail(q, plan_layer_launch(q), r, t);
+  std::lock_guard<std::mutex> lock(mu);
+  if (memo.size() > 256) memo.clear();
+  return memo[key] = out;
+}
+
+}
diff --git a/deepcgp_amd/csrc/head_units_dev.h b/deepcgp_amd/csrc/head_units_dev.h
--- a/deepcgp_amd/csrc/head_units_dev.h
+++ b/deepcgp_amd/csrc/head_units_dev.h
@@ -20,8 +20,8 @@
 #define HU_EXPN 4
 #endif
 #define HU_LDX(i) (COH ? __hip_atomic_load(Xn + (i), __ATOMIC_RELAXED, __HIP_MEMORY_SCOPE_AGENT) : Xn[i])
-template <int NK4, int TL, int WMODE, int NT, bool COH = false>
-__device__ __forceinline__ void head_units_body(const __attribute__((address_space(4))) HeadUnitsArgs& a, const int block) {
+template <int NK4, int TL, int WMODE, int NT, bool COH = false, bool SEL = false>
+__device__ __forceinline__ void head_units_body(const __attribute__((address_space(4))) HeadUnitsArgs& a, const int block, const int sel_sg = 0, const int sel_u = 0) {
   extern __shared__ __attribute__((aligned(16))) double smem[];
   constexpr bool WRITE = WMODE == 1 || WMODE == 2;
   constexpr bool KEEP = WMODE == 3;
@@ -43,14 +43,16 @@
   const char* imgb = reinterpret_cast<const char*>(img);
   const int tid = threadIdx.x, lane = tid & 63, lrow = lane >> 4, lcol = lane & 15;
   const int wave = __builtin_amdgcn_readfirstlane(tid >> 6);
-  int sg = 0;
-#pragma unroll
-  for (int q = 1; q < 6; ++q)
-    if (q < a.nseg && block >= a.seg[q].wg0) sg = q;
+  int sg = SEL ? sel_sg : 0;
+  if constexpr (!SEL) {
+#pragma unroll
+    for (int q = 1; q < 6; ++q)
+      if (q < a.nseg && block >= a.seg[q].wg0) sg = q;
+  }
   const int seg_kind = a.seg[sg].kind, seg_T = a.seg[sg].T, seg_C = a.seg[sg].C;
-  const int wloc = block - a.seg[sg].wg0, wpi = a.seg[sg].wpi;
-  const int nloc = wloc / wpi, bw = wloc - nloc * wpi;
-  const int n = a.seg[sg].img0 + nloc;
+  const int wloc = SEL ? 0 : block - a.seg[sg].wg0, wpi = SEL ? 1 : a.seg[sg].wpi;
+  const int nloc = SEL ? 0 : wloc / wpi, bw = wloc - nloc * wpi;
+  const int n = SEL ? block : a.seg[sg].img0 + nloc;
   const double* __restrict__ Xn = a.X + (long)((a.n0 + n) % a.n_mod) * HWC;
   auto ldi = [&](int byte_off) { return *reinterpret_cast<const double*>(imgb + byte_off); };
   long long* const tr = (a.trace && block < a.trace_wgs) ? a.trace + ((long)block * WPG + wave) * 8 : nullptr;
@@ -139,7 +141,7 @@
 
   stamp(3);
   const int seg_upw = a.seg[sg].upw;
-  int u = WPG * seg_upw * bw + ((wave + n) & (WPG - 1));
+  int u = SEL ? sel_u : WPG * seg_upw * bw + ((wave + n) & (WPG - 1));
   const int n_units = seg_kind == 1 ? seg_C : (WRITE ? a.nfm * a.st_split : a.nfm);
   if (u >= n_units) {
     if (tr && lane == 0) tr[6] = (long long)wall_clock64();
diff --git a/deepcgp_amd/csrc/layer.h b/deepcgp_amd/csrc/layer.h
--- a/deepcgp_amd/csrc/layer.h
+++ b/deepcgp_amd/csrc/layer.h
@@ -113,6 +113,7 @@
   int n_items = 0;
   int pre_D = 0, pre_whole = 0;
   int head_n = 0;
+  int tail_parts = 0, tail_upp = 0, tail_n = 0;
   unsigned* head_flag = nullptr; unsigned head_epoch = 0;
   HeadUnitsArgs head;
 };
@@ -131,6 +132,8 @@
 int conv_fused(dcgp_ctx* ctx, const ConvFusedArgs& a);
 int conv_fused_rides_head(const dcgp_ctx* ctx, const ConvFusedArgs& a, bool keeps_state, bool head_form, long head_HWC, long head_lds, long head_nfm, bool in_flight,
                            bool chain_beside);
+int conv_fused_head_tail(const dcgp_ctx* ctx, const ConvFusedArgs& a, bool keeps_state, bool head_form, long head_HWC, long head_lds, long head_nfm, long head_n_kd,
+                         bool in_flight, bool chain_beside, int* n_rows);
 
 int kl_layer(dcgp_ctx* ctx, const GpMats& g, const double* Lp, const double* LpinvT, int white, const char* ws_prefix,
              double* kl4);
diff --git a/deepcgp_amd/csrc/layer_impl.h b/deepcgp_amd/csrc/layer_impl.h
--- a/deepcgp_amd/csrc/layer_impl.h
+++ b/deepcgp_amd/csrc/layer_impl.h
@@ -316,7 +316,7 @@
                  const double* z, uint64_t seed, uint32_t stream_id, double jitter, double* out_sample, double* out_mean,
                  double* out_var, const std::string& pfx, hipEvent_t factor_done = nullptr,
                                hipEvent_t prep_done = nullptr, int phase = 3, bool keep_state = true, const RngMap* rmap = nullptr,
-                               int planned_one_launch = -1, const HeadUnitsArgs* ride_head = nullptr, int ride_rows = 0) {
+                               int planned_one_launch = -1, const HeadUnitsArgs* ride_head = nullptr, int ride_rows = 0, int ride_tail = 0) {
   const int Mp = L.Mp, P = L.v.P;
   const long Kc = (long)rows * P;
   if (Kc > 0x7fffff00L) return ctx_fail(ctx, DCGP_ERR_ARG, "conv layer: %ld patch columns exceed the 32-bit tile index", Kc);
@@ -348,10 +348,10 @@
       }
       if (prep_done) HIP_TRY(ctx, hipStreamWaitEvent(ctx->stream, prep_done, 0));
       else if (factor_done) HIP_TRY(ctx, hipStreamWaitEvent(ctx->stream, factor_done, 0));
-      if (ride_head) { fa.head = *ride_head; fa.head_n = ride_rows; }
+      if (ride_head) { fa.head = *ride_head; fa.head_n = ride_rows; fa.tail_parts = ride_tail; }
       if (!L.mean_W && !L.mix_W) return conv_fused(ctx, fa);
-      if (ride_head && ride_rows > 0 && L.mix_W) return ctx_fail(ctx, DCGP_ERR_ARG, "conv layer: a mixed layer cannot carry the head's rows");
-      if (ride_head && ride_rows > 0) return ctx_fail(ctx, DCGP_ERR_ARG, "conv layer: a layer with a mean filter cannot carry the head's rows");
+      if (ride_head && (ride_rows > 0 || ride_tail > 0) && L.mix_W) return ctx_fail(ctx, DCGP_ERR_ARG, "conv layer: a mixed layer cannot carry the head's rows");
+      if (ride_head && (ride_rows > 0 || ride_tail > 0)) return ctx_fail(ctx, DCGP_ERR_ARG, "conv layer: a layer with a mean filter cannot carry the head's rows");
       DCGP_TRY(conv_fused(ctx, fa));
       if (L.mix_W)
         DCGP_TRY(mix_forward(ctx, L.mix_W, L.R, L.Rout, out_sample, out_mean, out_var, 0, Kc, rep, rep_stride, out_stride, mix_sample, mix_mean, mix_var));
@@ -428,7 +428,7 @@
 static inline int head_forward(dcgp_ctx* ctx, LayerState& L, const double* X, int rows, int n_mod, double* kd, double* out_mean,
                  double* out_var, const std::string& pfx, hipEvent_t factor_done = nullptr,
                                hipEvent_t prep_done = nullptr, int sweep_mode = 0, bool* early_done = nullptr,
-                               bool keep_k = false, KlOffer* kl = nullptr, int kzx_done = 0) {
+                               bool keep_k = false, KlOffer* kl = nullptr, int kzx_done = 0, bool sweep_done = false) {
   const int Mp = L.Mp;
   const long ldb = col_ld(rows);
   if (sweep_mode != 2) L.kfull_ready = false;
@@ -469,6 +469,7 @@
         if (sweep_mode != 0 || h.kfull || h.nseg < 2 || h.seg[0].kind != 0)
           return ctx_fail(ctx, DCGP_ERR_ARG, "head: its Kzx rows were run by the layer kernel, but the sweep is not the one that was planned");
         if (kzx_done > rows) return ctx_fail(ctx, DCGP_ERR_ARG, "head: more Kzx rows done than the head has");
+        if (sweep_done && kzx_done != rows) return ctx_fail(ctx, DCGP_ERR_ARG, "head: the whole sweep is done, but not every Kzx row");
         const int gone = h.seg[0].wpi * kzx_done;
         for (int q = 1; q < h.nseg; ++q) h.seg[q].wg0 -= gone;
         h.n_wgs -= gone;
@@ -478,7 +479,10 @@
           --h.nseg;
         }
       }
-      if (sweep_mode != 2) DCGP_TRY(head_units(ctx, h));
+      if (sweep_done) {
+        if (!exp2_table(ctx)) return DCGP_ERR_ALLOC;
+        ++ctx->head_sweeps_skipped;
+      } else if (sweep_mode != 2) DCGP_TRY(head_units(ctx, h));
       if (sweep_mode == 1) {
         if (early_done) *early_done = true;
         return DCGP_OK;
@@ -500,7 +504,7 @@
       return finalize_layer(ctx, fa);
     }
   }
-  if (kzx_done) return ctx_fail(ctx, DCGP_ERR_ARG, "head: its Kzx rows were run by the layer kernel, but the head does not take the unit sweep");
+  if (kzx_done || sweep_done) return ctx_fail(ctx, DCGP_ERR_ARG, "head: its Kzx rows were run by the layer kernel, but the head does not take the unit sweep");
   if (sweep_mode == 1) return DCGP_OK;
   if (L.kernel_type == 0 && a.bk.type == 0 && head_cond_fused_ok(L.g) && !unfused) {
     const double* kdp = nullptr; int kd_n = 1; double kd_scale = 1.0;
diff --git a/deepcgp_amd/csrc/model.hip b/deepcgp_amd/csrc/model.hip
--- a/deepcgp_amd/csrc/model.hip
+++ b/deepcgp_amd/csrc/model.hip
@@ -130,6 +130,7 @@
   ChainMode chain;
   ForkMark mark = ForkMark::BehindFirstLayer;
   int ride_layer = -1, ride_rows = 0;
+  int ride_tail = 0;
   bool chain_beside() const { return chain_s != main_s; }
 };
 struct StepIn { const double* X; int N, S; const double* const* zs; uint64_t seed; int dedup; bool need_kl; };
@@ -167,9 +168,17 @@
     HeadUnitsArgs h = head_sweep_shape(ctx, Lh, nullptr, rows_out, rows_out, nullptr, col_ld(rows_out));
     head_units_plan(&h);
     const bool form = head_sweep_rides_form(ctx, Lh, h) && !(m->keep_state && m->grad_follows);
-    if (li > 0 || p.first_one_launch)
-      p.ride_rows = conv_fused_rides_head(ctx, fa, m->keep_state, form, h.HWC, (long)head_units_lds(h), h.nfm, pipelined, p.chain_beside() && !p.reuse);
-    if (p.ride_rows > 0) p.ride_layer = li;
+    if (li > 0 || p.first_one_launch) {
+      static double kzx_placeholder;
+      HeadUnitsArgs hk = h;
+      hk.kzx = &kzx_placeholder;
+      head_units_plan(&hk);
+      int tail_rows = 0;
+      p.ride_tail = conv_fused_head_tail(ctx, fa, m->keep_state, form, h.HWC, (long)head_units_lds(h), h.nfm, hk.n_kd, pipelined, p.chain_beside() && !p.reuse, &tail_rows);
+      if (p.ride_tail > 0) p.ride_rows = tail_rows;
+      else p.ride_rows = conv_fused_rides_head(ctx, fa, m->keep_state, form, h.HWC, (long)head_units_lds(h), h.nfm, pipelined, p.chain_beside() && !p.reuse);
+    }
+    if (p.ride_rows > 0 || p.ride_tail > 0) p.ride_layer = li;
   }
   return p;
 }
@@ -246,11 +255,15 @@
       if (!B) return DCGP_ERR_ALLOC;
       ride = head_sweep_shape(ctx, Lh, o.sample, out_rows, out_rows, B, ldh);
       head_units_plan(&ride);
+      if (p.ride_tail > 0) {
+        ride.kd = (double*)ws_get(ctx, "kdiag_partial", (size_t)out_rows * ride.n_kd * sizeof(double));
+        if (!ride.kd) return DCGP_ERR_ALLOC;
+      }
     }
     DCGP_TRY(conv_forward(ctx, L, F, rows, n_mod, expand ? in.S : 1, (long)in.N * lat_width, z, in.seed, (uint32_t)(li + 1 + (sharded ? 0 : 64 * ctx->rank)),
                           m->jitter, o.sample, m->keep_outputs ? o.mean : nullptr, m->keep_outputs ? o.var : nullptr, pfx,
                           fdone, pdone, phase, m->keep_state, &rm, li == 0 ? (int)p.first_one_launch : -1,
-                          (li == p.ride_layer && (phase & 2)) ? &ride : nullptr, p.ride_rows));
+                          (li == p.ride_layer && (phase & 2)) ? &ride : nullptr, p.ride_rows, p.ride_tail));
     *out_rows_p = out_rows;
     return DCGP_OK;
   }
@@ -259,7 +272,8 @@
   DCGP_TRY(ensure(ctx, &m->d_kd, &m->kd_cap, (size_t)rows));
   DCGP_TRY(head_forward(ctx, L, F, rows, n_mod, m->d_kd, o.mean, o.var, pfx, fdone, pdone,
                         phase == 1 ? 1 : (phase == 2 && *head_swept ? 2 : 0), phase == 1 ? head_swept : nullptr,
-                        m->keep_state && m->grad_follows, kl, (p.ride_layer == li - 1 && p.ride_layer >= 0) ? p.ride_rows : 0));
+                        m->keep_state && m->grad_follows, kl, (p.ride_layer == li - 1 && p.ride_layer >= 0) ? (p.ride_tail > 0 ? rows : p.ride_rows) : 0,
+                        p.ride_layer == li - 1 && p.ride_layer >= 0 && p.ride_tail > 0));
   *out_rows_p = rows;
   if (phase != 1 && m->keep_outputs) {
     size_t n = (size_t)rows * L.R;
diff --git a/deepcgp_amd/device.py b/deepcgp_amd/device.py
--- a/deepcgp_amd/device.py
+++ b/deepcgp_amd/device.py
@@ -163,6 +163,8 @@
     "dcgp_debug_plan_gemm": [_vp, _i, _vp, _i],
     "dcgp_debug_head_ride": [_vp, _vp],
     "dcgp_debug_plan_head_ride": [_vp, _i, _vp, _i, C.c_longlong, _vp, _i],
+    "dcgp_debug_head_tail": [_vp, _vp],
+    "dcgp_debug_plan_head_tail": [_vp, _i, _vp, _i, _vp, _i, C.c_longlong, _vp, _i],
     "dcgp_debug_comm_gate": [_vp, _i, _ip],
     "dcgp_debug_mfma_f64_rate": [_vp, _dp],
     "dcgp_debug_store_rate": [_vp, _i, _i, _i, _dp],
diff --git a/include/dcgp.h b/include/dcgp.h
--- a/include/dcgp.h
+++ b/include/dcgp.h
@@ -262,6 +262,9 @@
 int dcgp_debug_plan_gemm(const long long* query, int n_query, long long* plan, int n_plan);
 int dcgp_debug_head_ride(dcgp_ctx* ctx, long long* out2);
 int dcgp_debug_plan_head_ride(const long long* query, int n_query, const long long* ride, int n_ride, long long row, long long* out, int n_out);
+int dcgp_debug_head_tail(dcgp_ctx* ctx, long long* out4);
+int dcgp_debug_plan_head_tail(const long long* query, int n_query, const long long* ride, int n_ride, const long long* tail, int n_tail, long long item,
+                              long long* out, int n_out);
 int dcgp_debug_mfma_f64_rate(dcgp_ctx* ctx, double* tflops_out);
 int dcgp_debug_store_rate(dcgp_ctx* ctx, int N, int P, int M, double* gbs_out);
 int dcgp_debug_set_sweep_trace(dcgp_ctx* ctx, long long* buf_dev, long n_workgroups, const char* family );
```
